# rock-slam/slam-pose_estimation

Hardware: NVIDIA B200
Metric: PoseUKF predict+update filter-steps/s (higher is better)
Workload: dtype f64

## Files before the change

slam_pose_estimation_b200/csrc/simt.cuh:

```cuda
#ifndef UKFB_SIMT_CUH
#define UKFB_SIMT_CUH

#ifndef UKFB_SIMT_EMU

#include <cuda_runtime.h>
#include <math.h>
#include <stdint.h>

#define UKFB_HD __host__ __device__ __forceinline__
#define UKFB_D __device__ __forceinline__
#define UKFB_DNI __device__ __noinline__
#define UKFB_GLOBAL __global__
#define UKFB_GRID_CONSTANT __grid_constant__
#define UKFB_CONSTANT __constant__
#define UKFB_LDCG(p) __ldcg(p)
#define UKFB_LAUNCH_BOUNDS(t, b) __launch_bounds__(t, b)
#define UKFB_SMEM_DECL extern __shared__ __align__(16) double ukfb_smem[];
#define UKFB_LDG(p) __ldg(p)
#define UKFB_UNROLL _Pragma("unroll")
#define UKFB_NOUNROLL _Pragma("unroll 1")

namespace ukfb {

UKFB_D void ukfb_sincos(double x, double* s, double* c) { sincos(x, s, c); }

UKFB_D void prefetch_l2(const void* p) { asm volatile("prefetch.global.L2 [%0];" ::"l"(p)); }

UKFB_D double warp_shfl(double v, int src) { return __shfl_sync(0xffffffffu, v, src); }

UKFB_D int hi_word(double x) { return __double2hiint(x); }

UKFB_D void pdl_launch_dependents() { asm volatile("griddepcontrol.launch_dependents;" ::: "memory"); }
UKFB_D void tile_done_add(unsigned long long* counter)
{
    asm volatile("red.release.gpu.global.add.u64 [%0], %1;" ::"l"(counter), "l"(1ull) : "memory");
}
UKFB_D void tile_done_wait(const unsigned long long* counter, unsigned long long need)
{
    unsigned long long v;
    for (unsigned spins = 0;; ++spins) {
        asm volatile("ld.acquire.gpu.global.u64 %0, [%1];" : "=l"(v) : "l"(counter) : "memory");
        if (v >= need) break;
        if (spins > 40000000u) __trap();
        __nanosleep(200);
    }
}

UKFB_D void warp_dmma(double& c0, double& c1, double a, double b)
{
    asm volatile("mma.sync.aligned.m8n8k4.row.col.f64.f64.f64.f64 {%0,%1}, {%2}, {%3}, {%0,%1};"
                 : "+d"(c0), "+d"(c1)
                 : "d"(a), "d"(b));
}

#ifndef UKFB_SEED_REFINEMENTS
#define UKFB_SEED_REFINEMENTS 2
#endif
UKFB_D double fast_rcp(double x)
{
    double y;
    asm("rcp.approx.ftz.f64 %0, %1;" : "=d"(y) : "d"(x));
    double e = fma(-x, y, 1.0);
    y = fma(y, e, y);
#if UKFB_SEED_REFINEMENTS >= 3
    e = fma(-x, y, 1.0);
    y = fma(y, e, y);
#endif
    e = fma(-x, y, 1.0);
    return fma(y, e, y);
}

UKFB_D void fast_sqrt_rsqrt(double x, double& s, double& r)
{
    double y;
    asm("rsqrt.approx.ftz.f64 %0, %1;" : "=d"(y) : "d"(x));
    double g = x * y, h = 0.5 * y;
    double e = fma(-g, h, 0.5);
    g = fma(g, e, g), h = fma(h, e, h);
#if UKFB_SEED_REFINEMENTS >= 3
    e = fma(-g, h, 0.5);
    g = fma(g, e, g), h = fma(h, e, h);
#endif
    e = fma(-g, h, 0.5);
    g = fma(g, e, g), h = fma(h, e, h);
    const double d = fma(-g, g, x);
    s = fma(d, h, g);
    r = h + h;
}

}

#else

#include <cmath>
#include <cstdint>

#include "simt_emu_rt.hpp"

#define UKFB_HD inline
#define UKFB_D inline
#define UKFB_DNI inline
#define UKFB_GLOBAL
#define UKFB_GRID_CONSTANT
#define UKFB_CONSTANT static const
#define UKFB_LDCG(p) (*(p))
#define UKFB_LAUNCH_BOUNDS(t, b)
#define UKFB_SMEM_DECL double* ukfb_smem = ::simt_emu::smem_base();
#define UKFB_LDG(p) (*(p))
#define UKFB_UNROLL
#define UKFB_NOUNROLL

namespace ukfb {
using std::atan;
using std::fabs;
using std::fma;
using std::sqrt;
inline void prefetch_l2(const void*) {}
inline int hi_word(double x)
{
    long long b;
    static_assert(sizeof(b) == sizeof(x), "");
    __builtin_memcpy(&b, &x, sizeof(b));
    return int(b >> 32);
}
inline void pdl_launch_dependents() {}
inline void tile_done_add(unsigned long long* counter) { __atomic_fetch_add(counter, 1ull, __ATOMIC_RELEASE); }
inline void tile_done_wait(const unsigned long long* counter, unsigned long long need)
{
    while (__atomic_load_n(counter, __ATOMIC_ACQUIRE) < need) {
    }
}
inline void ukfb_sincos(double x, double* s, double* c)
{
    *s = std::sin(x);
    *c = std::cos(x);
}
inline double warp_shfl(double v, int src)
{
    double* x = ::simt_emu::warp_xchg();
    const int lane = threadIdx.x & 31;
    x[lane] = v;
    __syncwarp();
    const double r = x[src & 31];
    __syncwarp();
    return r;
}
inline void warp_dmma(double& c0, double& c1, double a, double b)
{
    double* x = ::simt_emu::warp_xchg();
    const int lane = threadIdx.x & 31;
    x[lane] = a;
    x[32 + lane] = b;
    __syncwarp();
    const int row = lane >> 2, col = 2 * (lane & 3);
    for (int k = 0; k < 4; ++k) {
        c0 += x[row * 4 + k] * x[32 + col * 4 + k];
        c1 += x[row * 4 + k] * x[32 + (col + 1) * 4 + k];
    }
    __syncwarp();
}
inline double fast_rcp(double x) { return 1.0 / x; }
inline void fast_sqrt_rsqrt(double x, double& s, double& r)
{
    s = std::sqrt(x);
    r = 1.0 / s;
}
}

#endif

#endif
```

slam_pose_estimation_b200/csrc/ukf_batch.cu:

```cuda
#include <cuda_runtime.h>

#include <algorithm>
#include <cassert>
#include <cfloat>
#include <cmath>
#include <vector>
#include <cstdarg>
#include <cstdio>
#include <cstring>
#include <new>
#include <condition_variable>
#include <functional>
#include <mutex>
#include <string>
#include <thread>
#include <utility>

#include "ukf_device.cuh"
#include "ukf_thread.cuh"
#include "ukf_index.cuh"
#ifndef UKFB_DEFAULT_PREFETCH_BYTES
#define UKFB_DEFAULT_PREFETCH_BYTES 128
#endif
#ifndef UKFB_DEFAULT_WPB
// ... 332 lines not shown
        double v = 0.0;
        if (k < MU)
            v = mu[b * MU + k];
        else {
            const int e = k - MU;
            int r = 0;
            while ((r + 1) * (r + 2) / 2 <= e) ++r;
            const int c = e - r * (r + 1) / 2;
            v = sigma[(b * n + r) * n + c];
        }
        state[rec_index(tiled, b, k, REC)] = v;
    }
}

__global__ void unpack_mu_kernel(const double* __restrict__ state, double* __restrict__ mu, long long B, int MU, int REC, int tiled)
{
    const long long total = B * MU;
    for (long long i = blockIdx.x * (long long)blockDim.x + threadIdx.x; i < total; i += (long long)gridDim.x * blockDim.x) {
        const long long b = i / MU;
        const int k = int(i - b * MU);
        mu[i] = state[rec_index(tiled, b, k, REC)];
    }
}

__global__ void unpack_sigma_kernel(const double* __restrict__ state, double* __restrict__ sigma, long long B, int n, int MU, int REC, int tiled)
{
    const long long total = B * n * n;
    for (long long i = blockIdx.x * (long long)blockDim.x + threadIdx.x; i < total; i += (long long)gridDim.x * blockDim.x) {
        const long long b = i / (n * n);
        const int e = int(i - b * n * n);
        int r = e / n, c = e - (e / n) * n;
        if (c > r) {
            const int t = r;
            r = c;
            c = t;
        }
        sigma[i] = state[rec_index(tiled, b, MU + tri(r, c), REC)];
    }
}

__global__ void pack_rbs_kernel(double* __restrict__ state, const double* __restrict__ rbs, long long B, int tiled)
{
    const long long total = B * PoseF::REC;
    for (long long i = blockIdx.x * (long long)blockDim.x + threadIdx.x; i < total; i += (long long)gridDim.x * blockDim.x) {
        const long long b = i / PoseF::REC;
        const int k = int(i - b * PoseF::REC);
        const double* r = rbs + b * UKFB_RBS_DOUBLES;
        double v = 0.0;
        if (k < PoseF::MU)
            v = r[k];
        else {
            const int e = k - PoseF::MU;
            int row = 0;
            while ((row + 1) * (row + 2) / 2 <= e) ++row;
            const int col = e - row * (row + 1) / 2;
            if (row / 3 == col / 3) v = r[13 + (row / 3) * 9 + (row % 3) * 3 + (col % 3)];
        }
        state[rec_index(tiled, b, k, PoseF::REC)] = v;
    }
}

__global__ void unpack_rbs_kernel(const double* __restrict__ state, double* __restrict__ rbs, long long B, int tiled)
{
    const long long total = B * UKFB_RBS_DOUBLES;
    for (long long i = blockIdx.x * (long long)blockDim.x + threadIdx.x; i < total; i += (long long)gridDim.x * blockDim.x) {
        const long long b = i / UKFB_RBS_DOUBLES;
        const int k = int(i - b * UKFB_RBS_DOUBLES);
        double v;
        if (k >= 7 && k < 10) {
            double q[4], bv[3], nv[3];
            for (int j = 0; j < 4; ++j) q[j] = state[rec_index(tiled, b, 3 + j, PoseF::REC)];
            for (int j = 0; j < 3; ++j) bv[j] = state[rec_index(tiled, b, 7 + j, PoseF::REC)];
            quat_rotate(q, bv, nv);
            v = nv[k - 7];
        } else if (k < PoseF::MU)
            v = state[rec_index(tiled, b, k, PoseF::REC)];
        else {
            const int blk = (k - 13) / 9, e = (k - 13) % 9;
            int row = blk * 3 + e / 3, col = blk * 3 + e % 3;
            if (col > row) {
                const int t = row;
                row = col;
                col = t;
            }
            v = state[rec_index(tiled, b, PoseF::MU + tri(row, col), PoseF::REC)];
        }
        rbs[i] = v;
    }
}

__global__ void pack_q_kernel(double* __restrict__ Qp, const double* __restrict__ Q, long long count, int n, int LP)
{
    const long long total = count * LP;
    for (long long i = blockIdx.x * (long long)blockDim.x + threadIdx.x; i < total; i += (long long)gridDim.x * blockDim.x) {
        const long long b = i / LP;
        const int e = int(i - b * LP);
        int r = 0;
        while ((r + 1) * (r + 2) / 2 <= e) ++r;
        const int c = e - r * (r + 1) / 2;
        Qp[i] = Q[(b * n + r) * n + c];
    }
}

__global__ void unpack_q_kernel(const double* __restrict__ Qp, double* __restrict__ Q, long long count, int n, int LP, long long q_stride)
{
    const long long total = count * n * n;
    for (long long i = blockIdx.x * (long long)blockDim.x + threadIdx.x; i < total; i += (long long)gridDim.x * blockDim.x) {
        const long long b = i / (n * n);
        const int e = int(i - b * n * n);
        int r = e / n, c = e - (e / n) * n;
        if (c > r) {
            const int t = r;
            r = c;
            c = t;
        }
        Q[i] = Qp[b * q_stride + tri(r, c)];
    }
}

template <typename T>
__global__ void fill_kernel(T* __restrict__ dst, long long count, T v)
{
    for (long long i = blockIdx.x * (long long)blockDim.x + threadIdx.x; i < count; i += (long long)gridDim.x * blockDim.x) dst[i] = v;
}

__global__ void eye3_kernel(double* __restrict__ dst, long long count)
{
    for (long long i = blockIdx.x * (long long)blockDim.x + threadIdx.x; i < count; i += (long long)gridDim.x * blockDim.x)
        dst[i] = ((i % 9) % 4 == 0) ? 1.0 : 0.0;
}

__global__ void store_vec3_kernel(double* __restrict__ dst_mu, double* __restrict__ dst_cov, const double* __restrict__ mu,
                                  const double* __restrict__ cov, long long cov_stride, const uint8_t* __restrict__ mask,
                                  uint32_t* __restrict__ status, int check, long long B)
{
    for (long long b = blockIdx.x * (long long)blockDim.x + threadIdx.x; b < B; b += (long long)gridDim.x * blockDim.x) {
        if (mask && !mask[b]) continue;
        const double m0 = mu[b * 3], m1 = mu[b * 3 + 1], m2 = mu[b * 3 + 2];
        double c[9];
        for (int i = 0; i < 9; ++i) c[i] = cov ? cov[b * cov_stride + i] : ((i % 4 == 0) ? 1.0 : 0.0);
        if (check) {
            bool ok = isfinite(m0) && isfinite(m1) && isfinite(m2);
            for (int i = 0; i < 9; ++i) ok = ok && isfinite(c[i]);
            if (!ok) {
                status[b] |= UKFB_STATUS_NONFINITE_MEAS;
                continue;
            }
        }
        dst_mu[b * 3] = m0, dst_mu[b * 3 + 1] = m1, dst_mu[b * 3 + 2] = m2;
        if (dst_cov)
            for (int i = 0; i < 9; ++i) dst_cov[b * 9 + i] = c[i];
    }
}

__global__ void rotation_rate_kernel(const double* __restrict__ state, const double* __restrict__ gyro, double e0, double e1,
                                     double e2, const double* __restrict__ ori_params, double* __restrict__ out, long long B, int tiled)
{
    for (long long b = blockIdx.x * (long long)blockDim.x + threadIdx.x; b < B; b += (long long)gridDim.x * blockDim.x) {
        double q[4];
        for (int i = 0; i < 4; ++i) q[i] = state[rec_index(tiled, b, i, OriF::REC)];
        double e[3] = {e0, e1, e2};
        if (ori_params) e[0] = ori_params[b * 5 + 2], e[1] = ori_params[b * 5 + 3], e[2] = ori_params[b * 5 + 4];
        double r[3];
        quat_inv_rotate(q, e, r);
        for (int i = 0; i < 3; ++i) out[b * 3 + i] = gyro[b * 3 + i] - state[rec_index(tiled, b, 7 + i, OriF::REC)] - r[i];
    }
}

__global__ void ori_default_imu_kernel(const double* __restrict__ state, double* __restrict__ acc, double* __restrict__ gyro,
                                       long long B, int tiled)
{
    for (long long b = blockIdx.x * (long long)blockDim.x + threadIdx.x; b < B; b += (long long)gridDim.x * blockDim.x) {
        acc[b * 3] = 0.0, acc[b * 3 + 1] = 0.0, acc[b * 3 + 2] = state[rec_index(tiled, b, 13, OriF::REC)];
        gyro[b * 3] = gyro[b * 3 + 1] = gyro[b * 3 + 2] = 0.0;
    }
}

__global__ void status_summary_kernel(const uint32_t* __restrict__ status, long long B, long long* __restrict__ out)
{
    long long n = 0;
    unsigned bits = 0;
    for (long long b = blockIdx.x * (long long)blockDim.x + threadIdx.x; b < B; b += (long long)gridDim.x * blockDim.x) {
        const uint32_t s = status[b];
        n += s != 0;
        bits |= s;
    }
    for (int o = 16; o; o >>= 1) {
        n += __shfl_xor_sync(0xffffffffu, n, o);
        bits |= __shfl_xor_sync(0xffffffffu, bits, o);
    }
    if ((threadIdx.x & 31) == 0) {
        if (n) atomicAdd(reinterpret_cast<unsigned long long*>(out), (unsigned long long)n);
        if (bits) atomicOr(reinterpret_cast<unsigned long long*>(out + 1), (unsigned long long)bits);
    }
}

__global__ void __launch_bounds__(256) dfma_peak_kernel(double* out, int iters, double a, double b)
{
    double x0 = threadIdx.x, x1 = x0 + 1, x2 = x0 + 2, x3 = x0 + 3, x4 = x0 + 4, x5 = x0 + 5, x6 = x0 + 6, x7 = x0 + 7;
    for (int i = 0; i < iters; ++i) {
#pragma unroll
        for (int u = 0; u < 8; ++u) {
            x0 = fma(x0, a, b), x1 = fma(x1, a, b), x2 = fma(x2, a, b), x3 = fma(x3, a, b);
            x4 = fma(x4, a, b), x5 = fma(x5, a, b), x6 = fma(x6, a, b), x7 = fma(x7, a, b);
        }
    }
    const double s = ((x0 + x1) + (x2 + x3)) + ((x4 + x5) + (x6 + x7));
    if (s == 12345.678) out[0] = s;
}

static inline int grid_for(long long count, int block = 256)
{
    long long g = (count + block - 1) / block;
    if (g < 1) g = 1;
    if (g > 148 * 16) g = 148 * 16;
    return int(g);
}

struct EnvKnobs {
    int fast_wpb;
    long smem_pad_kb;
    int prefetch_bytes;
    long long prefetch_tiles;
    bool overlap;
    int overlap_max_waves;
    int overlap_min_waves_pct;
    EnvKnobs()
    {
        const char* e = getenv("UKFB_FAST_WPB");
        const int v = e ? atoi(e) : UKFB_DEFAULT_WPB;
        fast_wpb = (v == 1 || v == 2 || v == 4) ? v : UKFB_DEFAULT_WPB;
        e = getenv("UKFB_SMEM_PAD_KB");
        smem_pad_kb = e ? atol(e) : 0;
        e = getenv("UKFB_PREFETCH_BYTES");
        prefetch_bytes = e && atoi(e) >= 8 ? atoi(e) : UKFB_DEFAULT_PREFETCH_BYTES;
        e = getenv("UKFB_PREFETCH_TILES");
        prefetch_tiles = e ? atoll(e) : -1;
        e = getenv("UKFB_OVERLAP_LAUNCHES");
        overlap = e ? atoi(e) != 0 : true;
        e = getenv("UKFB_OVERLAP_MAX_WAVES");
        overlap_max_waves = e && atoi(e) > 0 ? atoi(e) : 12;
        e = getenv("UKFB_OVERLAP_MIN_WAVES_PCT");
        overlap_min_waves_pct = e ? atoi(e) : 100;
    }
};
static const EnvKnobs& knobs()
{
    static const EnvKnobs k;
    return k;
}

static std::mutex g_attr_mu;
template <class K>
static cudaError_t ensure_smem_attr(K kernel, int device, size_t smem)
{
    static std::vector<std::pair<const void*, int>> done;
    const std::pair<const void*, int> key(reinterpret_cast<const void*>(kernel), device);
    std::lock_guard<std::mutex> lock(g_attr_mu);
    for (const auto& d : done)
        if (d == key) return cudaSuccess;
    cudaError_t e = cudaFuncSetAttribute(kernel, cudaFuncAttributeMaxDynamicSharedMemorySize, int(smem));
    if (e == cudaSuccess) done.push_back(key);
    return e;
}

template <class F, int G, int WPB, int MINB>
static cudaError_t launch_step_t(const ukfb_handle* h, const StepParams& p)
{
    const size_t smem = sizeof(double) * WPB * Smem<F, G>::TOTAL;
    cudaError_t e = ensure_smem_attr(ukf_step_kernel<F, G, WPB, MINB>, h->device, smem);
    if (e != cudaSuccess) return e;
    const long long per_block = (long long)WPB * G;
    const long long grid = (p.B + per_block - 1) / per_block;
    ukf_step_kernel<F, G, WPB, MINB><<<unsigned(grid), WPB * 32, smem, h->stream>>>(p);
    return cudaGetLastError();
}

template <class F>
static cudaError_t launch_step_f(const ukfb_handle* h, const StepParams& p)
{
    switch (h->G * 100 + h->WPB * 10 + h->MINB) {
        case 443: return launch_step_t<F, 4, 4, 3>(h, p);
        case 444: return launch_step_t<F, 4, 4, 4>(h, p);
        case 1642: return launch_step_t<F, 16, 4, 2>(h, p);
        case 1652: return launch_step_t<F, 16, 5, 2>(h, p);
        case 842: return launch_step_t<F, 8, 4, 2>(h, p);
        case 844: return launch_step_t<F, 8, 4, 4>(h, p);
        default: return launch_step_t<F, 8, 4, 3>(h, p);
    }
}

template <class F>
static cudaError_t launch_thread_f(const ukfb_handle* h, const StepParams& p)
{
    const size_t smem = sizeof(double) * TSmem<F>::TOTAL;
    cudaError_t e = ensure_smem_attr(ukf_thread_kernel<F>, h->device, smem);
    if (e != cudaSuccess) return e;
    const long long grid = (p.B + TILE - 1) / TILE;
    ukf_thread_kernel<F><<<unsigned(grid), TILE, smem, h->stream>>>(p);
    return cudaGetLastError();
}

template <class K>
static cudaError_t launch_fast(K kernel, K kernel_overlap, int per_lane, ukfb_handle* h, const StepParams& p, ukfb_handle::FastCfg& cfg)
{
    const EnvKnobs& kn = knobs();
    const int wpb = kn.fast_wpb;
    const size_t smem = sizeof(double) * per_lane * TILE * wpb + size_t(kn.smem_pad_kb) * 1024;
    if (!cfg.attr_set) {
        cudaError_t e = ensure_smem_attr(kernel, h->device, smem);
        if (e == cudaSuccess) e = ensure_smem_attr(kernel_overlap, h->device, smem);
        if (e != cudaSuccess) return e;
        cfg.attr_set = true;
    }
    const long long tiles = (p.B + TILE - 1) / TILE;
    const long long grid = (tiles + wpb - 1) / wpb;
    StepParams q = p;
    if (cfg.prefetch_tiles < 0) {
        int per_sm = 0, sms = 0;
        if (cudaOccupancyMaxActiveBlocksPerMultiprocessor(&per_sm, kernel, TILE * wpb, smem) != cudaSuccess) per_sm = 0;
        if (cudaDeviceGetAttribute(&sms, cudaDevAttrMultiProcessorCount, h->device) != cudaSuccess) sms = 0;
        cfg.resident_warps = (long long)per_sm * wpb * sms;
        long long r = kn.prefetch_tiles;
        if (r < 0) {
            r = cfg.resident_warps / 4;
            if (r < 32 && per_sm > 0) r = 32;
        }
        cfg.prefetch_tiles = r > 0 ? r : 0;
    }
    q.prefetch_tiles = cfg.prefetch_tiles;
    q.prefetch_bytes = kn.prefetch_bytes;
    const bool overlap = kn.overlap && cfg.resident_warps > 0 && grid * wpb * 100 > kn.overlap_min_waves_pct * cfg.resident_warps &&
                         grid * wpb <= kn.overlap_max_waves * cfg.resident_warps;
    q.tile_done = overlap ? h->tile_done : nullptr;
    q.launch_seq = h->fast_launches + 1;
    cudaLaunchConfig_t lc;
    memset(&lc, 0, sizeof(lc));
    lc.gridDim = dim3(unsigned(grid));
    lc.blockDim = dim3(TILE * wpb);
    lc.dynamicSmemBytes = smem;
    lc.stream = h->stream;
    cudaLaunchAttribute at[1];
    at[0].id = cudaLaunchAttributeProgrammaticStreamSerialization;
    at[0].val.programmaticStreamSerializationAllowed = 1;
    lc.attrs = at;
    lc.numAttrs = overlap ? 1 : 0;
    const cudaError_t e = cudaLaunchKernelEx(&lc, overlap ? kernel_overlap : kernel, q);
    if (e != cudaSuccess) return e;
    if (overlap) h->fast_launches++;
    return cudaGetLastError();
}

static cudaError_t launch_pose_fast(ukfb_handle* h, const StepParams& p, bool may_have_orientation_meas)
{
    if (may_have_orientation_meas) return launch_fast(ukf_pose_fast_kernel<true, false>, ukf_pose_fast_kernel<true, true>, PF_PER_LANE, h, p, h->fast_cfg[1]);
    return launch_fast(ukf_pose_fast_kernel<false, false>, ukf_pose_fast_kernel<false, true>, PF_PER_LANE, h, p, h->fast_cfg[0]);
}

static cudaError_t launch_ori_fast(ukfb_handle* h, const StepParams& p)
{
    if (p.ori_params) return launch_fast(ukf_ori_fast_kernel<true, false>, ukf_ori_fast_kernel<true, true>, OF_PER_LANE, h, p, h->fast_cfg[1]);
    return launch_fast(ukf_ori_fast_kernel<false, false>, ukf_ori_fast_kernel<false, true>, OF_PER_LANE, h, p, h->fast_cfg[0]);
}

static int launch_step(ukfb_handle* h, const StepParams& p)
{
    cudaError_t e;
    if (h->tiled && h->fast && h->kind == UKFB_POSE) {
        bool ori_meas = p.do_update && (p.kind == UKFB_MEAS_POSE_ORIENTATION || p.kind == -2 || p.events);
        if (p.do_update && p.tick_kinds) ori_meas = h->tick_kinds_have_orientation;
        e = launch_pose_fast(h, p, ori_meas);
    }
    else if (h->tiled && h->fast)
        e = launch_ori_fast(h, p);
    else if (h->tiled)
        e = h->kind == UKFB_POSE ? launch_thread_f<PoseF>(h, p) : launch_thread_f<OriF>(h, p);
    else
        e = h->kind == UKFB_POSE ? launch_step_f<PoseF>(h, p) : launch_step_f<OriF>(h, p);
    if (e != cudaSuccess) return fail(UKFB_ERR_CUDA, "ukf_step_kernel launch: %s", cudaGetErrorString(e));
    h->launches++;
    return UKFB_OK;
}

static StepParams base_params(const ukfb_handle* h)
{
    StepParams p;
    memset(&p, 0, sizeof(p));
    p.state = h->state;
    p.Q = h->Q;
    p.q_stride = h->q_per_filter ? h->LP : 0;
    p.q_diagonal = h->q_per_filter ? 0 : h->q_diagonal;
    p.B = h->B;
    p.status = h->status;
    p.t_last = h->t_last;
    p.hist = h->hist;
    p.min_dt = h->min_dt;
    p.max_dt = h->max_dt;
    p.acc_mu = h->acc_mu;
    p.acc_cov = h->acc_cov;
    p.gyro_mu = h->gyro_mu;
    p.neg_inv_tau_g = -1.0 / h->tau_g;
    p.neg_inv_tau_a = -1.0 / h->tau_a;
    p.earth[0] = h->earth[0], p.earth[1] = h->earth[1], p.earth[2] = h->earth[2];
    p.kind = -1;
    p.K = 1;
    p.gate_d2 = h->gate_d2;
    p.ori_params = h->ori_params;
    return p;
}

static bool kind_ok(const ukfb_handle* h, int kind)
{
    if (h->kind == UKFB_POSE) return kind >= 0 && kind <= 8;
    return kind == UKFB_MEAS_ORI_VELOCITY;
}

#define NEED_INIT_AS(h, who) \
    if (!(h)->initialized) return fail(UKFB_ERR_NOT_INITIALIZED, "%s: filter not initialized", who)
#define NEED_INIT(h) NEED_INIT_AS(h, __func__)

extern "C" int ukfb_create(int filter_kind, int64_t batch, int device, ukfb_handle** out)
{
    if (!out) return fail(UKFB_ERR_INVALID, "ukfb_create: out is null");
    *out = nullptr;
    if (filter_kind != UKFB_POSE && filter_kind != UKFB_ORIENTATION) return fail(UKFB_ERR_INVALID, "ukfb_create: bad filter kind %d", filter_kind);
    if (batch < 1) return fail(UKFB_ERR_INVALID, "ukfb_create: batch must be >= 1");
    int ndev = 0;
    cudaError_t e = cudaGetDeviceCount(&ndev);
    if (e != cudaSuccess || ndev == 0)
        return fail(UKFB_ERR_CUDA, "ukfb_create: no CUDA device (%s); this engine has no CPU path", cudaGetErrorString(e));
    if (device < 0 || device >= ndev) return fail(UKFB_ERR_INVALID, "ukfb_create: device %d out of range (%d devices)", device, ndev);
    cudaDeviceProp prop;
    CU(cudaGetDeviceProperties(&prop, device));
    if (prop.major < 10) return fail(UKFB_ERR_CUDA, "ukfb_create: device %d is sm_%d%d; the kernels are built for sm_100a only", device, prop.major, prop.minor);

    ukfb_handle* h = new (std::nothrow) ukfb_handle;
    if (!h) return fail(UKFB_ERR_NOMEM, "ukfb_create: out of host memory");
    h->kind = filter_kind;
    h->device = device;
    h->B = batch;
    if (filter_kind == UKFB_POSE)
        h->n = PoseF::N, h->MU = PoseF::MU, h->LP = PoseF::LP, h->REC = PoseF::REC;
    else
        h->n = OriF::N, h->MU = OriF::MU, h->LP = OriF::LP, h->REC = OriF::REC;
    if (const char* g = getenv("UKFB_GROUP")) {
        const int G = atoi(g);
        if (G == 4 || G == 8 || G == 16) h->G = G;
    }
    if (const char* g = getenv("UKFB_KERNEL")) {
        h->tiled = strcmp(g, "warp") != 0;
        if (strcmp(g, "thread") == 0) h->fast = 0;
    }
    if (const char* g = getenv("UKFB_WARP_WPB")) h->WPB = atoi(g);
    if (const char* g = getenv("UKFB_MINB")) h->MINB = atoi(g);
    Bind bind_(h);
    if (!bind_.ok) {
        delete h;
        return fail(UKFB_ERR_CUDA, "ukfb_create: cudaSetDevice(%d) failed", device);
    }
#define CUH(call)                                                                     \
    do {                                                                              \
        cudaError_t e_ = (call);                                                      \
        if (e_ != cudaSuccess) {                                                      \
            fail(e_ == cudaErrorMemoryAllocation ? UKFB_ERR_NOMEM : UKFB_ERR_CUDA, "%s: %s", #call, cudaGetErrorString(e_)); \
            ukfb_destroy(h);                                                          \
            return e_ == cudaErrorMemoryAllocation ? UKFB_ERR_NOMEM : UKFB_ERR_CUDA; \
        }                                                                             \
    } while (0)
    const long long B = batch;
    CUH(cudaStreamCreateWithFlags(&h->stream, cudaStreamNonBlocking));
    const long long Bpad = (B + TILE - 1) / TILE * TILE;
    CUH(cudaMalloc(&h->state, sizeof(double) * Bpad * h->REC));
    CUH(cudaMalloc(&h->Q, sizeof(double) * h->LP));
    CUH(cudaMalloc(&h->status, sizeof(uint32_t) * B));
    CUH(cudaMalloc(&h->t_last, sizeof(long long) * B));
    CUH(cudaMalloc(&h->hist, sizeof(unsigned long long) * HIST_SLOTS * 8));
    CUH(cudaMalloc(&h->acc_mu, sizeof(double) * B * 3));
    CUH(cudaMalloc(&h->acc_cov, sizeof(double) * B * 9));
    CUH(cudaMalloc(&h->gyro_mu, sizeof(double) * B * 3));
    CUH(cudaMalloc(&h->summary, sizeof(long long) * 2));
    CUH(cudaMalloc(&h->tile_done, sizeof(unsigned long long) * (Bpad / TILE)));
    CUH(cudaMemsetAsync(h->tile_done, 0, sizeof(unsigned long long) * (Bpad / TILE), h->stream));
    CUH(cudaMemsetAsync(h->state, 0, sizeof(double) * Bpad * h->REC, h->stream));
    CUH(cudaMemsetAsync(h->status, 0, sizeof(uint32_t) * B, h->stream));
    CUH(cudaMemsetAsync(h->t_last, 0, sizeof(long long) * B, h->stream));
    CUH(cudaMemsetAsync(h->hist, 0, sizeof(unsigned long long) * HIST_SLOTS * 8, h->stream));
    CUH(cudaMemsetAsync(h->gyro_mu, 0, sizeof(double) * B * 3, h->stream));
    {
        double q[OriF::LP];
        for (int i = 0; i < OriF::LP; ++i) q[i] = 0.0;
        if (filter_kind == UKFB_POSE) {
            const double d[4] = {UKFB_POSE_Q_POSITION, UKFB_POSE_Q_ORIENTATION, UKFB_POSE_Q_VELOCITY, UKFB_POSE_Q_ANGULAR_VELOCITY};
            for (int i = 0; i < 12; ++i) q[tri(i, i)] = d[i / 3];
        }
        CUH(cudaMemcpyAsync(h->Q, q, sizeof(double) * h->LP, cudaMemcpyHostToDevice, h->stream));
        CUH(cudaStreamSynchronize(h->stream));
        h->q_diagonal = 2;
    }
    fill_kernel<double><<<grid_for(B * 3), 256, 0, h->stream>>>(h->acc_mu, B * 3, filter_kind == UKFB_POSE ? double(NAN) : 0.0);
    eye3_kernel<<<grid_for(B * 9), 256, 0, h->stream>>>(h->acc_cov, B * 9);
    for (int i = 0; i < 16; ++i) CUH(cudaEventCreate(&h->ev[i]));
    CUH(cudaGetLastError());
    CUH(cudaStreamSynchronize(h->stream));
#undef CUH
    *out = h;
    return UKFB_OK;
}

extern "C" int ukfb_create_sharded(int filter_kind, int64_t batch, const int* devices, int n_devices, ukfb_handle** out)
{
    if (!out) return fail(UKFB_ERR_INVALID, "ukfb_create_sharded: out is null");
    *out = nullptr;
    if (filter_kind != UKFB_POSE && filter_kind != UKFB_ORIENTATION) return fail(UKFB_ERR_INVALID, "ukfb_create_sharded: bad filter kind %d", filter_kind);
    if (n_devices < 1 || n_devices > 64) return fail(UKFB_ERR_INVALID, "ukfb_create_sharded: n_devices must be 1..64");
    if (batch < n_devices) return fail(UKFB_ERR_INVALID, "ukfb_create_sharded: batch must be >= n_devices (every shard holds at least one filter)");
    ukfb_handle* h = new (std::nothrow) ukfb_handle;
    if (!h) return fail(UKFB_ERR_NOMEM, "ukfb_create_sharded: out of host memory");
    h->kind = filter_kind;
    h->B = batch;
    if (filter_kind == UKFB_POSE)
        h->n = PoseF::N, h->MU = PoseF::MU, h->LP = PoseF::LP, h->REC = PoseF::REC;
    else
        h->n = OriF::N, h->MU = OriF::MU, h->LP = OriF::LP, h->REC = OriF::REC;
    const long long base = batch / n_devices, extra = batch % n_devices;
    h->first.assign(size_t(n_devices) + 1, 0);
    for (int i = 0; i < n_devices; ++i) h->first[size_t(i) + 1] = h->first[size_t(i)] + base + (i < extra ? 1 : 0);
    for (int i = 0; i < n_devices; ++i) {
        ukfb_handle* sh = nullptr;
        const int rc = ukfb_create(filter_kind, h->first[size_t(i) + 1] - h->first[size_t(i)], devices ? devices[i] : i, &sh);
        if (rc) {
            for (ukfb_handle* made : h->shards) ukfb_destroy(made);
            delete h;
            return rc;
        }
        h->shards.push_back(sh);
    }
    h->device = h->shards[0]->device;
    h->tiled = h->shards[0]->tiled, h->fast = h->shards[0]->fast;
    h->pool = new (std::nothrow) ShardPool(n_devices);
    if (!h->pool) {
        for (ukfb_handle* made : h->shards) ukfb_destroy(made);
        delete h;
        return fail(UKFB_ERR_NOMEM, "ukfb_create_sharded: out of host memory");
    }
    *out = h;
    return UKFB_OK;
}

extern "C" int ukfb_shard_count(const ukfb_handle* h) { return !h ? 0 : (is_sharded(h) ? int(h->shards.size()) : 1); }

extern "C" int ukfb_shard(ukfb_handle* h, int i, ukfb_handle** shard, int64_t* first, int64_t* count)
{
    if (!h) return fail(UKFB_ERR_INVALID, "ukfb_shard: null handle");
    const int n = ukfb_shard_count(h);
    if (i < 0 || i >= n) return fail(UKFB_ERR_INVALID, "ukfb_shard: shard %d out of range (%d shards)", i, n);
    if (shard) *shard = is_sharded(h) ? h->shards[size_t(i)] : h;
    if (first) *first = is_sharded(h) ? h->first[size_t(i)] : 0;
    if (count) *count = is_sharded(h) ? h->first[size_t(i) + 1] - h->first[size_t(i)] : h->B;
    return UKFB_OK;
}

extern "C" int ukfb_host_alloc(void** ptr, uint64_t bytes)
{
    if (!ptr || !bytes) return fail(UKFB_ERR_INVALID, "ukfb_host_alloc: bad argument");
    *ptr = nullptr;
    cudaError_t e = cudaHostAlloc(ptr, size_t(bytes), cudaHostAllocPortable);
    if (e != cudaSuccess) return fail(e == cudaErrorMemoryAllocation ? UKFB_ERR_NOMEM : UKFB_ERR_CUDA, "ukfb_host_alloc(%llu bytes): %s", (unsigned long long)bytes, cudaGetErrorString(e));
    return UKFB_OK;
}

extern "C" int ukfb_host_free(void* ptr)
{
    if (!ptr) return UKFB_OK;
    CU(cudaFreeHost(ptr));
    return UKFB_OK;
}

extern "C" int ukfb_destroy(ukfb_handle* h)
{
    if (!h) return UKFB_OK;
    if (is_sharded(h)) {
        delete h->pool;
        for (ukfb_handle* s : h->shards) ukfb_destroy(s);
        delete h;
        return UKFB_OK;
    }
    Bind bind_(h);
    if (h->stream) cudaStreamSynchronize(h->stream);
    cudaFree(h->state), cudaFree(h->Q), cudaFree(h->status), cudaFree(h->t_last), cudaFree(h->hist), cudaFree(h->tile_done), cudaFree(h->tick_kinds_dev);
    cudaFree(h->acc_mu), cudaFree(h->acc_cov), cudaFree(h->gyro_mu), cudaFree(h->stage), cudaFree(h->summary), cudaFree(h->ori_params);
    for (int k = 0; k < UKFB_MEAS_KIND_COUNT; ++k) cudaFree(h->meas_cov[k]);
    for (int i = 0; i < 16; ++i)
        if (h->ev[i]) cudaEventDestroy(h->ev[i]);
    if (h->pipe.made) {
        cudaStreamSynchronize(h->pipe.s_in), cudaStreamSynchronize(h->pipe.s_out);
        for (int i = 0; i < 2; ++i) {
            cudaFree(h->pipe.in[i]), cudaFree(h->pipe.out[i]);
            cudaEventDestroy(h->pipe.in_ready[i]), cudaEventDestroy(h->pipe.in_consumed[i]);
            cudaEventDestroy(h->pipe.out_ready[i]), cudaEventDestroy(h->pipe.out_drained[i]);
        }
        cudaStreamDestroy(h->pipe.s_in), cudaStreamDestroy(h->pipe.s_out);
    }
    if (h->stream) cudaStreamDestroy(h->stream);
    delete h;
    return UKFB_OK;
}

extern "C" int64_t ukfb_batch(const ukfb_handle* h) { return h ? h->B : 0; }
extern "C" int ukfb_dof(const ukfb_handle* h) { return h ? h->n : 0; }
extern "C" int ukfb_mu_size(const ukfb_handle* h) { return h ? h->MU : 0; }
extern "C" int ukfb_device(const ukfb_handle* h) { return h ? h->device : -1; }
extern "C" int ukfb_is_initialized(const ukfb_handle* h) { return h && h->initialized ? 1 : 0; }

static int initialize_dev(ukfb_handle* h, const double* d_mu, const double* d_sigma)
{
    pack_kernel<<<grid_for(h->B * h->REC), 256, 0, h->stream>>>(h->state, d_mu, d_sigma, h->B, h->n, h->MU, h->LP, h->REC, h->tiled);
    CU(cudaGetLastError());
    CU(cudaMemsetAsync(h->t_last, 0, sizeof(long long) * h->B, h->stream));
    if (h->kind == UKFB_ORIENTATION && h->first_init) {
        ori_default_imu_kernel<<<grid_for(h->B), 256, 0, h->stream>>>(h->state, h->acc_mu, h->gyro_mu, h->B, h->tiled);
        CU(cudaGetLastError());
    }
    h->first_init = false;
    h->initialized = true;
    return UKFB_OK;
}

extern "C" int ukfb_initialize(ukfb_handle* h, const double* mu, const double* sigma)
{
    CHECK_H(h);
    if (!mu || !sigma) return fail(UKFB_ERR_INVALID, "ukfb_initialize: null argument");
    if (is_sharded(h)) {
        const int rc = fan_out(h, [&](ukfb_handle* s_, long long f_, long long) { return ukfb_initialize(s_, mu + f_ * s_->MU, sigma + f_ * s_->n * s_->n); });
        if (rc == UKFB_OK) h->initialized = true;
        return rc;
    }
    const double *d_mu, *d_sigma;
    Staging st(h, false);
    st.in(&d_mu, mu, sizeof(double) * h->B * h->MU);
    st.in(&d_sigma, sigma, sizeof(double) * h->B * h->n * h->n);
    int rc = st.commit();
    if (!rc) rc = initialize_dev(h, d_mu, d_sigma);
    return rc ? rc : st.finish();
}

extern "C" int ukfb_initialize_from_body_states_dev(ukfb_handle* h, const double* d_rbs)
{
    CHECK_H(h);
    UKFB_NOT_SHARDED(h);
    if (h->kind != UKFB_POSE) return fail(UKFB_ERR_INVALID, "ukfb_initialize_from_body_states: BodyStateMeasurement belongs to PoseUKF");
    if (!d_rbs) return fail(UKFB_ERR_INVALID, "ukfb_initialize_from_body_states: null argument");
    pack_rbs_kernel<<<grid_for(h->B * h->REC), 256, 0, h->stream>>>(h->state, d_rbs, h->B, h->tiled);
    CU(cudaGetLastError());
    CU(cudaMemsetAsync(h->t_last, 0, sizeof(long long) * h->B, h->stream));
    h->first_init = false;
    h->initialized = true;
    return UKFB_OK;
}

extern "C" int ukfb_initialize_from_body_states(ukfb_handle* h, const double* rbs)
{
    CHECK_H(h);
    if (!rbs) return fail(UKFB_ERR_INVALID, "ukfb_initialize_from_body_states: null argument");
    if (is_sharded(h)) {
        if (h->kind != UKFB_POSE) return fail(UKFB_ERR_INVALID, "ukfb_initialize_from_body_states: BodyStateMeasurement belongs to PoseUKF");
// ... 1239 lines not shown
```

slam_pose_estimation_b200/csrc/ukf_pose_fast.cuh:

```cuda
#ifndef UKFB_POSE_FAST_CUH
#define UKFB_POSE_FAST_CUH

#include "ukf_thread.cuh"

namespace ukfb {

#define UKFB_PS(e) sm[(e) * TILE + lane]

#ifndef UKFB_PF_MEAN_UNROLL
#define UKFB_PF_MEAN_UNROLL 1
#endif
#ifndef UKFB_PF_COV_UNROLL
#define UKFB_PF_COV_UNROLL 1
#endif
#ifndef UKFB_PF_MIN_BLOCKS
#define UKFB_PF_MIN_BLOCKS 2
#endif
#ifndef UKFB_PF_MAX_THREADS
#define UKFB_PF_MAX_THREADS (4 * TILE)
#endif
#define UKFB_PRAGMA_(x) _Pragma(#x)
#ifdef UKFB_SIMT_EMU
#define UKFB_LOOP_UNROLL(n)
#else
// ... 50 lines not shown
    const double n2 = q[0] * q[0] + q[1] * q[1] + q[2] * q[2] + q[3] * q[3];
    return fabs(n2 - 1.0) <= PF_QNORM_TOL;
}

UKFB_D void pf_rotate(const double* q, const double* v, double* out)
{
    const double ux = fma(q[1], v[2], -(q[2] * v[1]));
    const double uy = fma(q[2], v[0], -(q[0] * v[2]));
    const double uz = fma(q[0], v[1], -(q[1] * v[0]));
    out[0] = fma(2.0, fma(q[3], ux, fma(q[1], uz, -(q[2] * uy))), v[0]);
    out[1] = fma(2.0, fma(q[3], uy, fma(q[2], ux, -(q[0] * uz))), v[1]);
    out[2] = fma(2.0, fma(q[3], uz, fma(q[0], uy, -(q[1] * ux))), v[2]);
}

UKFB_D void pf_matvec(const double* Rm, const double* v, double* out)
{
    out[0] = Rm[0] * v[0] + Rm[1] * v[1] + Rm[2] * v[2];
    out[1] = Rm[3] * v[0] + Rm[4] * v[1] + Rm[5] * v[2];
    out[2] = Rm[6] * v[0] + Rm[7] * v[1] + Rm[8] * v[2];
}

struct D2 {
    double a, b;
    UKFB_D D2() {}
    UKFB_D explicit D2(double x) : a(x), b(x) {}
    UKFB_D D2(double x, double y) : a(x), b(y) {}
};
UKFB_D D2 operator+(D2 x, D2 y) { return D2(x.a + y.a, x.b + y.b); }
UKFB_D D2 operator-(D2 x, D2 y) { return D2(x.a - y.a, x.b - y.b); }
UKFB_D D2 operator*(D2 x, D2 y) { return D2(x.a * y.a, x.b * y.b); }
UKFB_D D2 operator-(D2 x) { return D2(-x.a, -x.b); }
UKFB_D D2 operator+(D2 x, double y) { return D2(x.a + y, x.b + y); }
UKFB_D D2 operator-(D2 x, double y) { return D2(x.a - y, x.b - y); }
UKFB_D D2 operator*(D2 x, double y) { return D2(x.a * y, x.b * y); }
UKFB_D D2 operator*(double x, D2 y) { return D2(x * y.a, x * y.b); }
UKFB_D D2 operator+(double x, D2 y) { return D2(x + y.a, x + y.b); }
UKFB_D double tfma(double x, double y, double z) { return fma(x, y, z); }
UKFB_D D2 tfma(D2 x, D2 y, D2 z) { return D2(fma(x.a, y.a, z.a), fma(x.b, y.b, z.b)); }
UKFB_D D2 tfma(double x, D2 y, D2 z) { return D2(fma(x, y.a, z.a), fma(x, y.b, z.b)); }
UKFB_D D2 tfma(D2 x, double y, D2 z) { return D2(fma(x.a, y, z.a), fma(x.b, y, z.b)); }
UKFB_D D2 tfma(D2 x, D2 y, double z) { return D2(fma(x.a, y.a, z), fma(x.b, y.b, z)); }
UKFB_D D2 tfma(double x, D2 y, double z) { return D2(fma(x, y.a, z), fma(x, y.b, z)); }
UKFB_D D2 tfma(D2 x, double y, double z) { return D2(fma(x.a, y, z), fma(x.b, y, z)); }
UKFB_D D2 tfma(double x, double y, D2 z) { return D2(fma(x, y, z.a), fma(x, y, z.b)); }
UKFB_D bool all_le(D2 x, double lim) { return (x.a <= lim) && (x.b <= lim); }
#define UKFB_TPOLY5(C, v, v2) tfma(tfma(C[5], v, C[4]), (v2) * (v2), tfma(tfma(C[3], v, C[2]), v2, tfma(C[1], v, C[0])))

UKFB_D void pf_exp(const D2* v, double scale, D2* q, bool& slow)
{
    const double half = scale * 0.5;
    const D2 norm2 = v[0] * v[0] + v[1] * v[1] + v[2] * v[2];
    const D2 x2 = (half * half) * norm2;
    slow = slow || !(pf_exp_in_range(x2.a) && pf_exp_in_range(x2.b));
    const D2 x4 = x2 * x2;
    const D2 c = UKFB_TPOLY5(SO3_COS5_C, x2, x4);
    const D2 mult = UKFB_TPOLY5(SO3_SINC5_C, x2, x4) * half;
    q[0] = mult * v[0];
    q[1] = mult * v[1];
    q[2] = mult * v[2];
    q[3] = c;
}

UKFB_D D2 two_asin_over_s_poly(D2 y)
{
    const D2 y2 = y * y, y4 = y2 * y2;
    const D2 p01 = tfma(SO3_ASIN_C[1], y, SO3_ASIN_C[0]), p23 = tfma(SO3_ASIN_C[3], y, SO3_ASIN_C[2]);
    const D2 p45 = tfma(SO3_ASIN_C[5], y, SO3_ASIN_C[4]), p67 = tfma(SO3_ASIN_C[7], y, SO3_ASIN_C[6]);
    const D2 q0 = tfma(p23, y2, p01), q1 = tfma(p67, y2, p45);
    return tfma(tfma(SO3_ASIN_C[8], y4, q1), y4, q0);
}

UKFB_D void pf_log(const D2* q, D2* out, bool& slow)
{
    const D2 nv2 = q[0] * q[0] + q[1] * q[1] + q[2] * q[2];
    const D2 w = q[3];
    const D2 d = tfma(w, w, nv2) - 1.0;
    slow = slow || !(pf_log_in_range(w.a) && pf_log_in_range(w.b));
    const D2 s0 = two_asin_over_s_poly(tfma(-nv2, d, nv2));
    const D2 s = tfma(s0, -0.5 * d, s0);
    out[0] = s * q[0];
    out[1] = s * q[1];
    out[2] = s * q[2];
}

UKFB_D void pf_rotate(const D2* q, const D2* v, D2* out)
{
    const D2 ux = tfma(q[1], v[2], -(q[2] * v[1]));
    const D2 uy = tfma(q[2], v[0], -(q[0] * v[2]));
    const D2 uz = tfma(q[0], v[1], -(q[1] * v[0]));
    out[0] = tfma(2.0, tfma(q[3], ux, tfma(q[1], uz, -(q[2] * uy))), v[0]);
    out[1] = tfma(2.0, tfma(q[3], uy, tfma(q[2], ux, -(q[0] * uz))), v[1]);
    out[2] = tfma(2.0, tfma(q[3], uz, tfma(q[0], uy, -(q[1] * ux))), v[2]);
}

template <class B>
UKFB_D void quat_mul(const D2* a, const B* b, D2* r)
{
    r[3] = a[3] * b[3] - a[0] * b[0] - a[1] * b[1] - a[2] * b[2];
    r[0] = a[3] * b[0] + a[0] * b[3] + a[1] * b[2] - a[2] * b[1];
    r[1] = a[3] * b[1] + a[1] * b[3] + a[2] * b[0] - a[0] * b[2];
    r[2] = a[3] * b[2] + a[2] * b[3] + a[0] * b[1] - a[1] * b[0];
}
template <class B>
UKFB_D void quat_mul_conj(const D2* a, const B* b, D2* r)
{
    r[3] = a[3] * b[3] + a[0] * b[0] + a[1] * b[1] + a[2] * b[2];
    r[0] = -a[3] * b[0] + a[0] * b[3] - a[1] * b[2] + a[2] * b[1];
    r[1] = -a[3] * b[1] + a[1] * b[3] - a[2] * b[0] + a[0] * b[2];
    r[2] = -a[3] * b[2] + a[2] * b[3] - a[0] * b[1] + a[1] * b[0];
}

#ifndef UKFB_PF_WIDE_CALLS
#define UKFB_PF_WIDE_CALLS 1
#endif
constexpr double PF_EXP_WIDE_X2 = 10.24;
#ifndef UKFB_PF_WIDE_TRACE
#define UKFB_PF_WIDE_TRACE 1.0
#endif
constexpr double PF_WIDE_TRACE = UKFB_PF_WIDE_TRACE;
#define UKFB_TPOLY6(C, v, v2) \
    tfma(tfma(C[6], v2, tfma(C[5], v, C[4])), (v2) * (v2), tfma(tfma(C[3], v, C[2]), v2, tfma(C[1], v, C[0])))
UKFB_D bool all_le(double x, double lim) { return x <= lim; }
UKFB_D double v_sign(double w) { return w < 0.0 ? -1.0 : 1.0; }
UKFB_D D2 v_sign(D2 w) { return D2(v_sign(w.a), v_sign(w.b)); }
UKFB_D void v_sqrt_rsqrt(double x, double& sq, double& rs) { fast_sqrt_rsqrt(x, sq, rs); }
UKFB_D void v_sqrt_rsqrt(D2 x, D2& sq, D2& rs)
{
    fast_sqrt_rsqrt(x.a, sq.a, rs.a);
    fast_sqrt_rsqrt(x.b, sq.b, rs.b);
}

template <class V>
UKFB_D void pf_exp_wide(const V* v, double scale, V* q, bool& hard)
{
    const double half = scale * 0.5;
    const V norm2 = v[0] * v[0] + v[1] * v[1] + v[2] * v[2];
    const V x2 = (half * half) * norm2;
    hard = hard || !all_le(x2, PF_EXP_WIDE_X2);
    const V y2 = x2 * (1.0 / 64.0), y4 = y2 * y2;
    V w = UKFB_TPOLY6(SO3_COS_C, y2, y4);
    const V mult = UKFB_TPOLY6(SO3_SINC_C, y2, y4) * (half * 0.125);
    V a = mult * v[0], b = mult * v[1], c = mult * v[2];
    UKFB_UNROLL
    for (int k = 0; k < 3; ++k) {
        const V t = w + w, n = a * a + b * b + c * c;
        w = tfma(w, w, -n);
        a = t * a, b = t * b, c = t * c;
    }
    q[0] = a, q[1] = b, q[2] = c, q[3] = w;
}

template <class V>
UKFB_D void pf_log_wide(const V* q, V* out)
{
    V x = q[0], y = q[1], z = q[2], w = q[3];
    const V n2 = tfma(w, w, x * x + y * y + z * z);
    const V k = v_sign(w) * tfma(n2 - 1.0, -0.5, 1.0);
    x = x * k, y = y * k, z = z * k, w = w * k;
    UKFB_UNROLL
    for (int i = 0; i < 3; ++i) {
        V c, rc;
        v_sqrt_rsqrt((w + 1.0) * 0.5, c, rc);
        const V h = rc * 0.5;
        x = x * h, y = y * h, z = z * h, w = c;
    }
    const V nv2 = x * x + y * y + z * z;
    const V d = tfma(w, w, nv2) - 1.0;
    const V s0 = two_asin_over_s_poly(tfma(-nv2, d, nv2));
    const V sc = tfma(s0, -0.5 * d, s0) * 8.0;
    out[0] = sc * x, out[1] = sc * y, out[2] = sc * z;
}

template <class V> struct PfV3 { V v[3]; };
template <class V> struct PfQ4 { V q[4]; bool hard; };
#if UKFB_PF_WIDE_CALLS
template <class V>
UKFB_DNI PfQ4<V> pf_exp_wide_call(PfV3<V> v, double scale)
{
    PfQ4<V> r;
    r.hard = false;
    pf_exp_wide<V>(v.v, scale, r.q, r.hard);
    return r;
}
template <class V>
UKFB_DNI PfV3<V> pf_log_wide_call(PfQ4<V> q)
{
    PfV3<V> r;
    pf_log_wide<V>(q.q, r.v);
    return r;
}
template <class V>
UKFB_D void pf_exp_wide_shared(const V* v, double scale, V* q, bool& hard)
{
    PfV3<V> a;
    a.v[0] = v[0], a.v[1] = v[1], a.v[2] = v[2];
    const PfQ4<V> r = pf_exp_wide_call<V>(a, scale);
    q[0] = r.q[0], q[1] = r.q[1], q[2] = r.q[2], q[3] = r.q[3];
    hard = hard || r.hard;
}
template <class V>
UKFB_D void pf_log_wide_shared(const V* q, V* out)
{
    PfQ4<V> a;
    a.q[0] = q[0], a.q[1] = q[1], a.q[2] = q[2], a.q[3] = q[3], a.hard = false;
    const PfV3<V> r = pf_log_wide_call<V>(a);
    out[0] = r.v[0], out[1] = r.v[1], out[2] = r.v[2];
}
#else
template <class V>
UKFB_D void pf_exp_wide_shared(const V* v, double scale, V* q, bool& hard) { pf_exp_wide<V>(v, scale, q, hard); }
template <class V>
UKFB_D void pf_log_wide_shared(const V* q, V* out) { pf_log_wide<V>(q, out); }
#endif

template <bool WIDE>
UKFB_D void pf_exp1(const double* v, double scale, double* q, bool& slow)
{
    if (WIDE)
        pf_exp_wide_shared<double>(v, scale, q, slow);
    else
        pf_exp(v, scale, q, slow);
}
template <bool WIDE>
UKFB_D void pf_log1(const double* q, double* out, bool& slow)
{
    if (WIDE)
        pf_log_wide_shared<double>(q, out);
    else
        pf_log(q, out, slow);
}

template <int NCOL>
UKFB_D bool pf_cholesky(double* a)
{
    bool ok = true;
    UKFB_UNROLL
    for (int j = 0; j < NCOL; ++j) {
        double ajj = a[tri(j, j)];
        UKFB_UNROLL
        for (int k = 0; k < j; ++k) ajj -= a[tri(j, k)] * a[tri(j, k)];
        if (!pivot_ok(ajj)) {
            ok = false;
            ajj = 1.0;
        }
        double d, rinv;
        fast_sqrt_rsqrt(ajj, d, rinv);
        a[tri(j, j)] = d;
        UKFB_UNROLL
        for (int i = j + 1; i < 12; ++i) {
            double s = a[tri(i, j)];
            UKFB_UNROLL
            for (int k = 0; k < j; ++k) s -= a[tri(i, k)] * a[tri(j, k)];
            a[tri(i, j)] = s * rinv;
        }
    }
    return ok;
}

struct TrueT { static constexpr bool value = true; };
struct FalseT { static constexpr bool value = false; };

struct PoseMu {
    double p[3], q[4], v[3], w[3];
};

template <class F>
UKFB_D void prefetch_next_wave(const StepParams& p, long long tile, int lane)
{
    if (p.prefetch_tiles <= 0) return;
    const long long nt = tile + p.prefetch_tiles;
    if ((nt + 1) * TILE > p.B) return;
    const char* rec = reinterpret_cast<const char*>(p.state + nt * (TILE * F::REC));
    const int bytes = TILE * F::REC * int(sizeof(double));
    UKFB_NOUNROLL
    for (int o = lane * p.prefetch_bytes; o < bytes; o += TILE * p.prefetch_bytes) prefetch_l2(rec + o);
    const long long nb = nt * TILE;
    const int o = lane * p.prefetch_bytes;
    if (p.acc_mu && o < TILE * 24) prefetch_l2(reinterpret_cast<const char*>(p.acc_mu + nb * 3) + o);
    if (F::KIND == 1 && p.gyro_mu && o < TILE * 24) prefetch_l2(reinterpret_cast<const char*>(p.gyro_mu + nb * 3) + o);
    if (p.do_update && p.z && o < TILE * 8 * p.z_stride) prefetch_l2(reinterpret_cast<const char*>(p.z + nb * p.z_stride) + o);
    if (p.do_update && p.R && p.r_stride > 0 && o < TILE * 8 * p.r_stride)
        prefetch_l2(reinterpret_cast<const char*>(p.R + nb * p.r_stride) + o);
    if (p.do_predict && !p.time_mode && p.dt && o < TILE * 8 * p.dt_stride) prefetch_l2(reinterpret_cast<const char*>(p.dt + nb * p.dt_stride) + o);
}

template <bool WIDE, class V>
UKFB_D void pf_exp_t(const V* v, double scale, V* q, bool& flag)
{
    if (WIDE)
        pf_exp_wide_shared<V>(v, scale, q, flag);
    else
        pf_exp(v, scale, q, flag);
}
template <bool WIDE, class V>
UKFB_D void pf_log_t(const V* q, V* out, bool& flag)
{
    if (WIDE)
        pf_log_wide_shared<V>(q, out);
    else
        pf_log(q, out, flag);
}


template <bool WIDE>
UKFB_D void pf_point2(const D2* qs, const D2* ps, const D2* vs, const D2* ws, double dt, const double* ref_p, const double* ref_q,
                      D2* d, bool& slow)
{
    D2 rv[3], e[4], qn[4], r[4];
    pf_rotate(qs, vs, rv);
    pf_exp_t<WIDE>(ws, dt, e, slow);
    quat_mul(qs, e, qn);
    d[0] = tfma(dt, rv[0], ps[0]) - ref_p[0];
    d[1] = tfma(dt, rv[1], ps[1]) - ref_p[1];
    d[2] = tfma(dt, rv[2], ps[2]) - ref_p[2];
    quat_mul_conj(qn, ref_q, r);
    pf_log_t<WIDE>(r, d + 3, slow);
}

template <bool WIDE>
UKFB_D void pf_pair_a(const double* sm, int lane, int j, const PoseMu& m, const double* vm, double dt, const double* ref_p,
                      const double* ref_q, double* L, double* dpl, double* dmi, bool& slow)
{
    UKFB_UNROLL
    for (int i = 0; i < 12; ++i) L[i] = UKFB_PS(PF_LA + j * 12 + i);
    double e[4];
    pf_exp_t<WIDE>(L + 3, 1.0, e, slow);
    const double* q = m.q;
    const double t0 = e[0] * q[3] + e[1] * q[2] - e[2] * q[1];
    const double t1 = e[1] * q[3] + e[2] * q[0] - e[0] * q[2];
    const double t2 = e[2] * q[3] + e[0] * q[1] - e[1] * q[0];
    const double t3 = -(e[0] * q[0] + e[1] * q[1] + e[2] * q[2]);
    const D2 qs[4] = {D2(fma(e[3], q[0], t0), fma(e[3], q[0], -t0)), D2(fma(e[3], q[1], t1), fma(e[3], q[1], -t1)),
                      D2(fma(e[3], q[2], t2), fma(e[3], q[2], -t2)), D2(fma(e[3], q[3], t3), fma(e[3], q[3], -t3))};
    const D2 ps[3] = {D2(m.p[0] + L[0], m.p[0] - L[0]), D2(m.p[1] + L[1], m.p[1] - L[1]), D2(m.p[2] + L[2], m.p[2] - L[2])};
    const D2 vs[3] = {D2(vm[0] + L[6], vm[0] - L[6]), D2(vm[1] + L[7], vm[1] - L[7]), D2(vm[2] + L[8], vm[2] - L[8])};
    const D2 ws[3] = {D2(m.w[0] + L[9], m.w[0] - L[9]), D2(m.w[1] + L[10], m.w[1] - L[10]), D2(m.w[2] + L[11], m.w[2] - L[11])};
    D2 d[6];
    pf_point2<WIDE>(qs, ps, vs, ws, dt, ref_p, ref_q, d, slow);
    UKFB_UNROLL
    for (int i = 0; i < 6; ++i) dpl[i] = d[i].a, dmi[i] = d[i].b;
}

template <bool WIDE>
UKFB_D void pf_pair_b(const double* sm, int lane, int j, const double* Rm, const double* rw0, const double* c, double dt,
                      double* L, double* dopl, double* domi, double* wv, bool& slow)
{
    UKFB_UNROLL
    for (int i = 0; i < 6; ++i) L[i] = UKFB_PS(PF_LB + (j - 6) * 6 + i);
    double u[3], rv[3];
    pf_matvec(Rm, L + 3, u);
    pf_matvec(Rm, L, rv);
    wv[0] = dt * rv[0], wv[1] = dt * rv[1], wv[2] = dt * rv[2];
    const D2 rw[3] = {D2(rw0[0] + u[0], rw0[0] - u[0]), D2(rw0[1] + u[1], rw0[1] - u[1]), D2(rw0[2] + u[2], rw0[2] - u[2])};
    D2 e[4], r[4], d[3];
    pf_exp_t<WIDE>(rw, dt, e, slow);
    quat_mul(e, c, r);
    pf_log_t<WIDE>(r, d, slow);
    UKFB_UNROLL
    for (int i = 0; i < 3; ++i) dopl[i] = d[i].a, domi[i] = d[i].b;
}

template <bool WIDE>
UKFB_D void pf_pair_d(const double* sm, int lane, int j, const double* delta, const double* c, double* dp, double* dn, bool& slow)
{
    D2 v[3], e[4], r2[4], d[3];
    UKFB_UNROLL
    for (int i = 0; i < 3; ++i) {
        const double l = UKFB_PS(PF_LA + j * 12 + 3 + i);
        v[i] = D2(delta[3 + i] + l, delta[3 + i] - l);
    }
    pf_exp_t<WIDE>(v, 1.0, e, slow);
    quat_mul(e, c, r2);
    pf_log_t<WIDE>(r2, d, slow);
    UKFB_UNROLL
    for (int i = 0; i < 3; ++i) dp[i] = d[i].a, dn[i] = d[i].b;
}

#ifndef UKFB_PF_WIDE_COLUMN_N2
#define UKFB_PF_WIDE_COLUMN_N2 0.2
#endif
constexpr double PF_WIDE_COLUMN_N2 = UKFB_PF_WIDE_COLUMN_N2;
template <bool WIDE>
UKFB_D void pf_pair_a_sel(const double* sm, int lane, int j, const PoseMu& m, const double* vm, double dt, const double* ref_p,
                          const double* ref_q, double* L, double* dpl, double* dmi, bool& slow)
{
    if (!WIDE) {
        pf_pair_a<false>(sm, lane, j, m, vm, dt, ref_p, ref_q, L, dpl, dmi, slow);
        return;
    }
    const double l3 = UKFB_PS(PF_LA + j * 12 + 3), l4 = UKFB_PS(PF_LA + j * 12 + 4), l5 = UKFB_PS(PF_LA + j * 12 + 5);
    bool redo = l3 * l3 + l4 * l4 + l5 * l5 > PF_WIDE_COLUMN_N2;
    if (!redo) pf_pair_a<false>(sm, lane, j, m, vm, dt, ref_p, ref_q, L, dpl, dmi, redo);
    if (redo) pf_pair_a<true>(sm, lane, j, m, vm, dt, ref_p, ref_q, L, dpl, dmi, slow);
}
template <bool WIDE>
UKFB_D void pf_pair_b_sel(const double* sm, int lane, int j, const double* Rm, const double* rw0, const double* c, double dt,
                          double* L, double* dopl, double* domi, double* wv, bool& slow)
{
    if (!WIDE) {
        pf_pair_b<false>(sm, lane, j, Rm, rw0, c, dt, L, dopl, domi, wv, slow);
        return;
    }
    bool redo = false;
    pf_pair_b<false>(sm, lane, j, Rm, rw0, c, dt, L, dopl, domi, wv, redo);
    if (redo) pf_pair_b<true>(sm, lane, j, Rm, rw0, c, dt, L, dopl, domi, wv, slow);
}
template <bool WIDE>
UKFB_D void pf_pair_d_sel(const double* sm, int lane, int j, const double* delta, const double* c, double* dp, double* dn, bool& slow)
{
    if (!WIDE) {
        pf_pair_d<false>(sm, lane, j, delta, c, dp, dn, slow);
        return;
    }
    const double l3 = UKFB_PS(PF_LA + j * 12 + 3), l4 = UKFB_PS(PF_LA + j * 12 + 4), l5 = UKFB_PS(PF_LA + j * 12 + 5);
    bool redo = l3 * l3 + l4 * l4 + l5 * l5 > PF_WIDE_COLUMN_N2;
    if (!redo) pf_pair_d<false>(sm, lane, j, delta, c, dp, dn, redo);
    if (redo) pf_pair_d<true>(sm, lane, j, delta, c, dp, dn, slow);
}

#ifdef UKFB_SIMT_EMU
inline unsigned long long pf_fallbacks[5] = {0, 0, 0, 0, 0};
#define UKFB_PF_COUNT(i) __atomic_fetch_add(&pf_fallbacks[i], 1ull, __ATOMIC_RELAXED)
#else
#define UKFB_PF_COUNT(i)
#endif
struct PfLit {
    PoseMu m;
    uint32_t status;
    int passes;
};

UKFB_D void pf_mu_to_slots(double* loc, const PoseMu& m)
{
    typedef TSmem<PoseF> TS;
    UKFB_UNROLL
    for (int i = 0; i < 3; ++i) {
        loc[TS::OFF_MU + i] = m.p[i];
        loc[TS::OFF_MU + 7 + i] = m.v[i];
        loc[TS::OFF_MU + 10 + i] = m.w[i];
    }
    UKFB_UNROLL
    for (int i = 0; i < 4; ++i) loc[TS::OFF_MU + 3 + i] = m.q[i];
}

UKFB_D void pf_mu_from_slots(const double* loc, PoseMu& m)
{
    typedef TSmem<PoseF> TS;
    UKFB_UNROLL
    for (int i = 0; i < 3; ++i) {
        m.p[i] = loc[TS::OFF_MU + i];
        m.v[i] = loc[TS::OFF_MU + 7 + i];
        m.w[i] = loc[TS::OFF_MU + 10 + i];
    }
    UKFB_UNROLL
    for (int i = 0; i < 4; ++i) m.q[i] = loc[TS::OFF_MU + 3 + i];
}

UKFB_DNI PfLit pf_literal_predict(double* sig, const double* Qp, const double* acov, ModelArgs ma, PoseMu m)
{
    typedef TSmem<PoseF> TS;
    UKFB_PF_COUNT(0);
    double loc[TS::PER_LANE];
    PfLit r;
    r.m = m, r.passes = 0;
    pf_mu_to_slots(loc, m);
    if (!cholesky_thread<PoseF, 1>(sig, loc, 0)) {
        r.status = UKFB_STATUS_NOT_SPD;
        return r;
    }
    store_noise<PoseF, 1>(loc, 0, sig, Qp, acov, ma);
    r.status = mean_and_cov<PoseF, true, 1>(loc, 0, sig, ma, &r.passes);
    UKFB_UNROLL
    for (int i = 0; i < PoseF::MU; ++i) loc[TS::OFF_MU + i] = loc[TS::OFF_REF + i];
    pf_mu_from_slots(loc, r.m);
    return r;
}

struct PfDelta {
    double d[12];
};

UKFB_DNI PfLit pf_literal_update(double* sig, int kind, const double* zm, const double* Rm, int r_ld, ModelArgs ma, PoseMu m,
                                 PfDelta delta, bool first, double gate_d2)
{
    typedef TSmem<PoseF> TS;
    UKFB_PF_COUNT(first ? 1 : 2);
    double loc[TS::PER_LANE];
    PfLit r;
    r.m = m, r.passes = 0, r.status = 0;
    pf_mu_to_slots(loc, m);
    if (first) {
        if (!cholesky_thread<PoseF, 1>(sig, loc, 0)) {
            r.status = UKFB_STATUS_NOT_SPD;
            return r;
        }
        r.status = update_first_half<PoseF, 1>(loc, 0, sig, kind, zm, Rm, r_ld, gate_d2);
        if (r.status & UKFB_STATUS_MEAS_REJECTED) return r;
    } else {
        UKFB_UNROLL
        for (int i = 0; i < 12; ++i) loc[TS::OFF_DELTA + i] = delta.d[i];
    }
    if (!cholesky_thread<PoseF, 1>(sig, loc, 0)) {
        r.status |= UKFB_STATUS_NOT_SPD;
        return r;
    }
    r.status |= mean_and_cov<PoseF, false, 1>(loc, 0, sig, ma, &r.passes);
    UKFB_UNROLL
    for (int i = 0; i < PoseF::MU; ++i) loc[TS::OFF_MU + i] = loc[TS::OFF_REF + i];
    pf_mu_from_slots(loc, r.m);
    return r;
}

template <bool WIDE>
UKFB_D bool pf_predict(int q_diagonal, double* sm, int lane, double* sig, double* a, const double* Qp, const double* acov,
                       const ModelArgs& ma, PoseMu& m, bool to_smem, uint32_t& status, int& passes_out, bool& spd)
{
    const double dt = ma.dt;
    if (!WIDE && a[tri(3, 3)] + a[tri(4, 4)] + a[tri(5, 5)] > PF_WIDE_TRACE) return false;
    {
        spd = pf_cholesky<12>(a);
        if (!spd) return true;
        UKFB_UNROLL
        for (int j = 0; j < 6; ++j) {
            UKFB_UNROLL
            for (int i = 0; i < 12; ++i) UKFB_PS(PF_LA + j * 12 + i) = i >= j ? a[tri(i, j)] : 0.0;
        }
        UKFB_UNROLL
        for (int j = 6; j < 12; ++j) {
            UKFB_UNROLL
            for (int i = 6; i < 12; ++i) UKFB_PS(PF_LB + (j - 6) * 6 + (i - 6)) = i >= j ? a[tri(i, j)] : 0.0;
        }
    }
    bool slow = !pf_unit(m.q);
    double Rm[9];
    quat_matrix(m.q, Rm);
    double vm[3] = {m.v[0], m.v[1], m.v[2]};
    if (ma.has_acc) {
        vm[0] = fma(dt, ma.acc[0], vm[0]);
        vm[1] = fma(dt, ma.acc[1], vm[1]);
        vm[2] = fma(dt, ma.acc[2], vm[2]);
    }
    double rw0[3], p0n[3], q0n[4];
    {
        double rv0[3], e0[4];
        pf_matvec(Rm, vm, rv0);
        pf_matvec(Rm, m.w, rw0);
        p0n[0] = fma(dt, rv0[0], m.p[0]);
        p0n[1] = fma(dt, rv0[1], m.p[1]);
        p0n[2] = fma(dt, rv0[2], m.p[2]);
        pf_exp1<WIDE>(rw0, dt, e0, slow);
        quat_mul(e0, m.q, q0n);
    }
    double ref_p[3] = {p0n[0], p0n[1], p0n[2]};
    double ref_q[4] = {q0n[0], q0n[1], q0n[2], q0n[3]};

    int it = 0, passes = 0;
    while (true) {
        double md[6];
        double d0[6];
        {
            double r[4];
            d0[0] = p0n[0] - ref_p[0], d0[1] = p0n[1] - ref_p[1], d0[2] = p0n[2] - ref_p[2];
            quat_mul_conj(q0n, ref_q, r);
            pf_log1<WIDE>(r, d0 + 3, slow);
        }
        md[0] = 13.0 * d0[0], md[1] = 13.0 * d0[1], md[2] = 13.0 * d0[2];
        md[3] = d0[3], md[4] = d0[4], md[5] = d0[5];
        UKFB_LOOP_UNROLL(UKFB_PF_MEAN_UNROLL)
        for (int j = 0; j < 6; ++j) {
            double L[12], dpl[6], dmi[6];
            pf_pair_a_sel<WIDE>(sm, lane, j, m, vm, dt, ref_p, ref_q, L, dpl, dmi, slow);
            UKFB_UNROLL
            for (int i = 0; i < 6; ++i) md[i] += dpl[i] + dmi[i];
        }
        double c[4];
        quat_mul_conj(m.q, ref_q, c);
        UKFB_LOOP_UNROLL(UKFB_PF_MEAN_UNROLL)
        for (int j = 6; j < 12; ++j) {
            double L[6], dopl[3], domi[3], wv[3];
            pf_pair_b_sel<WIDE>(sm, lane, j, Rm, rw0, c, dt, L, dopl, domi, wv, slow);
            UKFB_UNROLL
            for (int i = 0; i < 3; ++i) md[3 + i] += dopl[i] + domi[i];
        }
        double n2 = 0.0;
        UKFB_UNROLL
        for (int i = 0; i < 6; ++i) {
            md[i] = div_ns<PoseF::NS>(md[i]);
            n2 += md[i] * md[i];
        }
        ref_p[0] += md[0], ref_p[1] += md[1], ref_p[2] += md[2];
        {
            double e[4], r[4];
            pf_exp1<WIDE>(md + 3, 1.0, e, slow);
            quat_mul(e, ref_q, r);
            ref_q[0] = r[0], ref_q[1] = r[1], ref_q[2] = r[2], ref_q[3] = r[3];
        }
        ++passes;
        if (slow || !(n2 > UKFB_MEAN_TOL * UKFB_MEAN_TOL)) break;
        if (++it >= UKFB_MEAN_MAX_IT) {
            status |= UKFB_STATUS_MEAN_NO_CONVERGE;
            break;
        }
    }
    if (slow) return false;

    double C[21], X[36];
    {
        double d0[6], r[4];
        d0[0] = p0n[0] - ref_p[0], d0[1] = p0n[1] - ref_p[1], d0[2] = p0n[2] - ref_p[2];
        quat_mul_conj(q0n, ref_q, r);
        pf_log1<WIDE>(r, d0 + 3, slow);
        UKFB_UNROLL
        for (int i = 0; i < 6; ++i) {
            UKFB_UNROLL
            for (int k = 0; k <= i; ++k) C[tri(i, k)] = d0[i] * d0[k];
        }
        UKFB_LOOP_UNROLL(UKFB_PF_COV_UNROLL)
        for (int j = 0; j < 6; ++j) {
            double L[12], dpl[6], dmi[6];
            pf_pair_a_sel<WIDE>(sm, lane, j, m, vm, dt, ref_p, ref_q, L, dpl, dmi, slow);
            UKFB_UNROLL
            for (int i = 0; i < 6; ++i) {
                UKFB_UNROLL
                for (int k = 0; k <= i; ++k) C[tri(i, k)] = fma(dpl[i], dpl[k], fma(dmi[i], dmi[k], C[tri(i, k)]));
            }
            UKFB_UNROLL
            for (int k = 0; k < 6; ++k) UKFB_PS(PF_LA + j * 12 + k) = dpl[k] - dmi[k];
        }
        double Xb[18];
        UKFB_UNROLL
        for (int i = 0; i < 18; ++i) Xb[i] = 0.0;
        double c[4];
        quat_mul_conj(m.q, ref_q, c);
        UKFB_LOOP_UNROLL(UKFB_PF_COV_UNROLL)
        for (int j = 6; j < 12; ++j) {
            double L[6], dpl[6], dmi[6], wv[3];
            pf_pair_b_sel<WIDE>(sm, lane, j, Rm, rw0, c, dt, L, dpl + 3, dmi + 3, wv, slow);
            UKFB_UNROLL
            for (int i = 0; i < 3; ++i) dpl[i] = d0[i] + wv[i], dmi[i] = d0[i] - wv[i];
            UKFB_UNROLL
            for (int i = 0; i < 6; ++i) {
                UKFB_UNROLL
                for (int k = 0; k <= i; ++k) C[tri(i, k)] = fma(dpl[i], dpl[k], fma(dmi[i], dmi[k], C[tri(i, k)]));
            }
            UKFB_UNROLL
            for (int k = 0; k < 3; ++k) {
                const double dd = dpl[3 + k] - dmi[3 + k];
                UKFB_UNROLL
                for (int i = 0; i < 6; ++i) Xb[i * 3 + k] = fma(L[i], dd, Xb[i * 3 + k]);
            }
        }
        if (slow) return false;
        UKFB_UNROLL
        for (int i = 0; i < 6; ++i) {
            UKFB_UNROLL
            for (int k = 0; k < 3; ++k) X[i * 6 + k] = 0.0, X[i * 6 + 3 + k] = Xb[i * 3 + k];
        }
        UKFB_UNROLL
        for (int j = 0; j < 6; ++j) {
            double dd[6];
            UKFB_UNROLL
            for (int k = 0; k < 6; ++k) dd[k] = UKFB_PS(PF_LA + j * 12 + k);
            UKFB_UNROLL
            for (int i = 0; i < 6; ++i) {
                const double l = UKFB_PS(PF_LA + j * 12 + 6 + i);
                UKFB_UNROLL
                for (int k = 0; k < 6; ++k) X[i * 6 + k] = fma(l, dd[k], X[i * 6 + k]);
            }
        }
        UKFB_UNROLL
        for (int j = 6; j < 9; ++j) {
            double Lc[6], rv[3];
            UKFB_UNROLL
            for (int i = 0; i < 6; ++i) Lc[i] = i >= j - 6 ? UKFB_PS(PF_LB + (j - 6) * 6 + i) : 0.0;
            pf_matvec(Rm, Lc, rv);
            UKFB_UNROLL
            for (int k = 0; k < 3; ++k) {
                const double dd = 2.0 * (dt * rv[k]);
                UKFB_UNROLL
                for (int i = j - 6; i < 6; ++i) X[i * 6 + k] = fma(Lc[i], dd, X[i * 6 + k]);
            }
        }
    }

    auto commit = [&](auto qv, auto iso) {
        const double scale = ma.has_acc ? 1.0 : dt;
        double nb[12], na[6];
        UKFB_UNROLL
        for (int i = 0; i < 12; ++i) nb[i] = 0.0;
        UKFB_UNROLL
        for (int i = 0; i < 6; ++i) na[i] = 0.0;
        if (!ma.has_acc && decltype(iso)::value) {
            nb[tri(0, 0)] = nb[tri(1, 1)] = nb[tri(2, 2)] = scale * qv(0, 0);
            nb[6 + tri(0, 0)] = nb[6 + tri(1, 1)] = nb[6 + tri(2, 2)] = scale * qv(3, 3);
        } else if (!ma.has_acc) {
            UKFB_UNROLL
            for (int blk = 0; blk < 2; ++blk) {
                const int off = blk * 3;
                double t[9];
                UKFB_UNROLL
                for (int r = 0; r < 3; ++r) {
                    UKFB_UNROLL
                    for (int k = 0; k < 3; ++k) {
                        double s = 0.0;
                        UKFB_UNROLL
                        for (int l = 0; l < 3; ++l) s += Rm[r * 3 + l] * (l >= k ? qv(off + l, off + k) : qv(off + k, off + l));
                        t[r * 3 + k] = s;
                    }
                }
                UKFB_UNROLL
                for (int r = 0; r < 3; ++r) {
                    UKFB_UNROLL
                    for (int cc = 0; cc <= r; ++cc) {
                        double s = 0.0;
                        UKFB_UNROLL
                        for (int k = 0; k < 3; ++k) s += t[r * 3 + k] * Rm[cc * 3 + k];
                        nb[blk * 6 + tri(r, cc)] = scale * s;
                    }
                }
            }
        } else {
            UKFB_UNROLL
            for (int r = 0; r < 3; ++r) {
                UKFB_UNROLL
                for (int cc = 0; cc <= r; ++cc) na[tri(r, cc)] = 2.0 * acov[r * 3 + cc];
            }
        }
        UKFB_UNROLL
        for (int i = 0; i < 12; ++i) {
            UKFB_UNROLL
            for (int k = 0; k <= i; ++k) {
                const int e = tri(i, k);
                double nz = scale * qv(i, k);
                if (i < 6 && i / 3 == k / 3) nz = ma.has_acc ? nz : nb[(i / 3) * 6 + tri(i % 3, k % 3)];
                if (i >= 6 && i < 9 && k >= 6) nz = ma.has_acc ? na[tri(i - 6, k - 6)] : nz;
                double s;
                if (i < 6)
                    s = fma(0.5, C[e], nz);
                else if (k < 6)
                    s = fma(0.5, X[(i - 6) * 6 + k], nz);
                else
                    s = sig[e * TILE] + nz;
                sig[e * TILE] = s;
                if (to_smem) UKFB_PS(e) = s;
            }
        }
    };
    if (q_diagonal == 2)
        commit([&](int i, int k) { return i == k ? UKFB_LDG(Qp + tri(i, i)) : 0.0; }, TrueT());
    else if (q_diagonal)
        commit([&](int i, int k) { return i == k ? UKFB_LDG(Qp + tri(i, i)) : 0.0; }, FalseT());
    else
        commit([&](int i, int k) { return UKFB_LDG(Qp + tri(i, k)); }, FalseT());
    m.p[0] = ref_p[0], m.p[1] = ref_p[1], m.p[2] = ref_p[2];
    m.q[0] = ref_q[0], m.q[1] = ref_q[1], m.q[2] = ref_q[2], m.q[3] = ref_q[3];
    m.v[0] = vm[0], m.v[1] = vm[1], m.v[2] = vm[2];
    passes_out = passes;
    return true;
}

UKFB_DNI PfLit pf_predict_slow(double* sm, int lane, double* sig, const double* Qp, const double* acov, ModelArgs ma, PoseMu m,
                               int to_smem, int q_diagonal, int* in_smem)
{
    {
        double a[PoseF::LP];
        UKFB_UNROLL
        for (int e = 0; e < PoseF::LP; ++e) a[e] = sig[e * TILE];
        PfLit r;
        r.m = m, r.status = 0, r.passes = 0;
        bool spd = true;
        if (pf_predict<true>(q_diagonal, sm, lane, sig, a, Qp, acov, ma, r.m, to_smem != 0, r.status, r.passes, spd)) {
            UKFB_PF_COUNT(3);
            if (!spd) r.status |= UKFB_STATUS_NOT_SPD;
            *in_smem = spd ? to_smem : 0;
            return r;
        }
    }
    *in_smem = 0;
    return pf_literal_predict(sig, Qp, acov, ma, m);
}

UKFB_D int pf_sel(int kind, int c)
{
    switch (kind) {
        case 0: return c;
        case 1: return c < 2 ? c : -1;
        case 2: return c == 0 ? 2 : -1;
        case 4: return 6 + c;
        case 5: return c < 2 ? 6 + c : -1;
        case 6: return c == 0 ? 8 : -1;
        case 7: return c == 0 ? 6 : (c == 1 ? 11 : -1);
        default: return 9 + c;
    }
}

UKFB_D double pf_mu_tangent(const PoseMu& m, int t)
{
    double r = m.p[0];
    r = t == 1 ? m.p[1] : r;
    r = t == 2 ? m.p[2] : r;
    r = t == 6 ? m.v[0] : r;
    r = t == 7 ? m.v[1] : r;
    r = t == 8 ? m.v[2] : r;
    r = t == 9 ? m.w[0] : r;
    r = t == 10 ? m.w[1] : r;
    r = t == 11 ? m.w[2] : r;
    return r;
}

template <bool WIDE>
UKFB_D bool pf_apply_delta(double* sm, int lane, double* sig, PoseMu& m, const double* delta, uint32_t& status, int& passes_out, int& stage)
{
    bool slow = !pf_unit(m.q);
    const bool off_sphere = slow;
    bool lost_factor = false;
    double e0[4], q0n[4];
    pf_exp1<WIDE>(delta + 3, 1.0, e0, slow);
    quat_mul(e0, m.q, q0n);
    double ref_q[4] = {q0n[0], q0n[1], q0n[2], q0n[3]};
    int it = 0, passes = 0;
    while (true) {
        double c[4], r[4], d0[3], md[3];
        quat_mul_conj(m.q, ref_q, c);
        quat_mul(e0, c, r);
        pf_log1<WIDE>(r, d0, slow);
        md[0] = 13.0 * d0[0], md[1] = 13.0 * d0[1], md[2] = 13.0 * d0[2];
        UKFB_NOUNROLL
        for (int j = 0; j < 6; ++j) {
            double dp[3], dn[3];
            pf_pair_d_sel<WIDE>(sm, lane, j, delta, c, dp, dn, slow);
            md[0] += dp[0] + dn[0], md[1] += dp[1] + dn[1], md[2] += dp[2] + dn[2];
        }
        double n2 = 0.0;
        UKFB_UNROLL
        for (int i = 0; i < 3; ++i) {
            md[i] = div_ns<PoseF::NS>(md[i]);
            n2 += md[i] * md[i];
        }
        {
            double e[4], rr[4];
            pf_exp1<WIDE>(md, 1.0, e, slow);
            quat_mul(e, ref_q, rr);
            ref_q[0] = rr[0], ref_q[1] = rr[1], ref_q[2] = rr[2], ref_q[3] = rr[3];
        }
        ++passes;
        if (slow || !(n2 > UKFB_MEAN_TOL * UKFB_MEAN_TOL)) break;
        if (++it >= UKFB_MEAN_MAX_IT) {
            status |= UKFB_STATUS_MEAN_NO_CONVERGE;
            break;
        }
    }
    double Coo[6], Xc[27];
    if (!slow) {
        double c[4], r[4], d0[3];
        quat_mul_conj(m.q, ref_q, c);
        quat_mul(e0, c, r);
        pf_log1<WIDE>(r, d0, slow);
        UKFB_UNROLL
        for (int i = 0; i < 3; ++i) {
            UKFB_UNROLL
            for (int k = 0; k <= i; ++k) Coo[tri(i, k)] = 13.0 * d0[i] * d0[k];
        }
        bool late = false;
        UKFB_NOUNROLL
        for (int j = 0; j < 6; ++j) {
            double dp[3], dn[3];
            pf_pair_d_sel<WIDE>(sm, lane, j, delta, c, dp, dn, late);
            UKFB_UNROLL
            for (int i = 0; i < 3; ++i) {
                UKFB_UNROLL
                for (int k = 0; k <= i; ++k) Coo[tri(i, k)] = fma(dp[i], dp[k], fma(dn[i], dn[k], Coo[tri(i, k)]));
            }
            UKFB_UNROLL
            for (int k = 0; k < 3; ++k) UKFB_PS(PF_LA + j * 12 + 3 + k) = dp[k] - dn[k];
        }
        slow = slow || late;
        lost_factor = late;
        UKFB_UNROLL
        for (int i = 0; i < 27; ++i) Xc[i] = 0.0;
        UKFB_UNROLL
        for (int j = 0; j < 6; ++j) {
            double dd[3];
            UKFB_UNROLL
            for (int k = 0; k < 3; ++k) dd[k] = UKFB_PS(PF_LA + j * 12 + 3 + k);
            UKFB_UNROLL
            for (int t = 0; t < 9; ++t) {
                const int row = t < 3 ? t : t + 3;
                if (row < j) continue;
                const double l = UKFB_PS(PF_LA + j * 12 + row);
                UKFB_UNROLL
                for (int k = 0; k < 3; ++k) Xc[t * 3 + k] = fma(l, dd[k], Xc[t * 3 + k]);
            }
        }
    }
    if (slow) {
        stage = (WIDE || lost_factor || off_sphere) ? 1 : 2;
        return false;
    }
    UKFB_UNROLL
    for (int i = 0; i < 3; ++i) {
        UKFB_UNROLL
        for (int k = 0; k <= i; ++k) sig[tri(3 + i, 3 + k) * TILE] = 0.5 * Coo[tri(i, k)];
        UKFB_UNROLL
        for (int t = 0; t < 3; ++t) sig[tri(3 + i, t) * TILE] = 0.5 * Xc[t * 3 + i];
        UKFB_UNROLL
        for (int t = 3; t < 9; ++t) sig[tri(t + 3, 3 + i) * TILE] = 0.5 * Xc[t * 3 + i];
    }
    UKFB_UNROLL
    for (int i = 0; i < 3; ++i) {
        m.p[i] += delta[i];
        m.v[i] += delta[6 + i];
        m.w[i] += delta[9 + i];
    }
    m.q[0] = ref_q[0], m.q[1] = ref_q[1], m.q[2] = ref_q[2], m.q[3] = ref_q[3];
    passes_out = passes;
    return true;
}

template <bool ORI_MEAS>
UKFB_D bool pf_update(double* sm, int lane, double* sig, int kind, const double* zm, const double* Rmeas, int r_ld, PoseMu& m,
                      double* delta, uint32_t& status, int& passes_out, bool& spd, double gate_d2, int& stage)
{
    stage = 0;
    const int m_dim = meas_dim(kind);
    int sel[3];
    UKFB_UNROLL
    for (int c = 0; c < 3; ++c) sel[c] = pf_sel(kind, c);

    double Sxz[36], S[9], innov[3];
    if (ORI_MEAS) {
        bool slow = !pf_unit(m.q);
        double a[PoseF::LP];
        UKFB_UNROLL
        for (int e = 0; e < PoseF::LP; ++e) a[e] = UKFB_PS(e);
        spd = pf_cholesky<12>(a);
        if (!spd) return true;
        constexpr int PF_E = 78;
        UKFB_UNROLL
        for (int j = 0; j < 6; ++j) {
            double e[4];
            const double Lo[3] = {j <= 3 ? a[tri(3, j <= 3 ? j : 3)] : 0.0, j <= 4 ? a[tri(4, j <= 4 ? j : 4)] : 0.0, a[tri(5, j)]};
            pf_exp(Lo, 1.0, e, slow);
            UKFB_UNROLL
            for (int i = 0; i < 4; ++i) UKFB_PS(PF_E + 4 * j + i) = e[i];
        }
        double zin[4];
        {
            const double v[3] = {zm[0], zm[1], zm[2]};
            so3_exp(v, 1.0, zin);
        }
        double zref[4] = {m.q[0], m.q[1], m.q[2], m.q[3]};
        int it = 0;
        while (!slow) {
            double c[4], d0[3], md[3];
            quat_mul_conj(m.q, zref, c);
            pf_log(c, d0, slow);
            md[0] = 13.0 * d0[0], md[1] = 13.0 * d0[1], md[2] = 13.0 * d0[2];
            UKFB_NOUNROLL
            for (int j = 0; j < 6; ++j) {
                D2 e[4], r2[4], d[3];
                UKFB_UNROLL
                for (int i = 0; i < 4; ++i) {
                    const double x = UKFB_PS(PF_E + 4 * j + i);
                    e[i] = D2(x, i < 3 ? -x : x);
                }
                quat_mul(e, c, r2);
                pf_log(r2, d, slow);
                md[0] += d[0].a + d[0].b, md[1] += d[1].a + d[1].b, md[2] += d[2].a + d[2].b;
            }
            UKFB_UNROLL
            for (int i = 0; i < 3; ++i) md[i] = div_ns<PoseF::NS>(md[i]);
            const double n2 = md[0] * md[0] + md[1] * md[1] + md[2] * md[2];
            {
                double e[4], rr[4];
                pf_exp(md, 1.0, e, slow);
                quat_mul(e, zref, rr);
                zref[0] = rr[0], zref[1] = rr[1], zref[2] = rr[2], zref[3] = rr[3];
            }
            if (!(n2 > UKFB_MEAN_TOL * UKFB_MEAN_TOL)) break;
            if (++it >= UKFB_MEAN_MAX_IT) {
                status |= UKFB_STATUS_MEAN_NO_CONVERGE;
                break;
            }
        }
        {
            double c[4], d0[3];
            quat_mul_conj(m.q, zref, c);
            pf_log(c, d0, slow);
            UKFB_UNROLL
            for (int r = 0; r < 3; ++r) {
                UKFB_UNROLL
                for (int cc = 0; cc < 3; ++cc) S[r * 3 + cc] = 13.0 * d0[r] * d0[cc];
            }
            UKFB_NOUNROLL
            for (int j = 0; j < 6; ++j) {
                D2 e[4], r2[4], d[3];
                UKFB_UNROLL
                for (int i = 0; i < 4; ++i) {
                    const double x = UKFB_PS(PF_E + 4 * j + i);
                    e[i] = D2(x, i < 3 ? -x : x);
                }
                quat_mul(e, c, r2);
                pf_log(r2, d, slow);
                UKFB_UNROLL
                for (int r = 0; r < 3; ++r) {
                    UKFB_UNROLL
                    for (int cc = 0; cc < 3; ++cc) S[r * 3 + cc] = fma(d[r].a, d[cc].a, fma(d[r].b, d[cc].b, S[r * 3 + cc]));
                    UKFB_PS(PF_E + 4 * j + r) = d[r].a - d[r].b;
                }
            }
            double r4[4];
            quat_mul_conj(zin, zref, r4);
            pf_log(r4, innov, slow);
        }
        if (slow) return false;
        UKFB_UNROLL
        for (int r = 0; r < 3; ++r) {
            UKFB_UNROLL
            for (int cc = 0; cc < 3; ++cc) S[r * 3 + cc] = fma(0.5, S[r * 3 + cc], Rmeas[r * r_ld + cc]);
        }
        UKFB_UNROLL
        for (int i = 0; i < 36; ++i) Sxz[i] = 0.0;
        UKFB_UNROLL
        for (int j = 0; j < 6; ++j) {
            UKFB_UNROLL
            for (int cc = 0; cc < 3; ++cc) {
                const double ddz = UKFB_PS(PF_E + 4 * j + cc);
                UKFB_UNROLL
                for (int i = j; i < 12; ++i) Sxz[i * 3 + cc] = fma(a[tri(i, j)], ddz, Sxz[i * 3 + cc]);
            }
        }
        UKFB_UNROLL
        for (int i = 0; i < 36; ++i) Sxz[i] *= 0.5;
    } else {
    UKFB_UNROLL
    for (int c = 0; c < 3; ++c) {
        const int s = sel[c] < 0 ? 0 : sel[c];
        const bool used = c < m_dim;
        UKFB_UNROLL
        for (int i = 0; i < 12; ++i) {
            const int e = i >= s ? tri(i, 0) + s : tri(s, 0) + i;
            const double x = UKFB_PS(e);
            Sxz[i * 3 + c] = used ? x : 0.0;
        }
        innov[c] = used ? zm[c] - pf_mu_tangent(m, s) : 0.0;
    }
    UKFB_UNROLL
    for (int a = 0; a < 3; ++a) {
        UKFB_UNROLL
        for (int c = 0; c < 3; ++c) {
            const int sa = sel[a] < 0 ? 0 : sel[a], sc = sel[c] < 0 ? 0 : sel[c];
            const int e = sa >= sc ? tri(sa, 0) + sc : tri(sc, 0) + sa;
            const bool used = a < m_dim && c < m_dim;
            const double x = UKFB_PS(e);
            S[a * 3 + c] = used ? x + Rmeas[a * r_ld + c] : (a == c ? 1.0 : 0.0);
        }
    }
    }
    double Si[9];
    {
        const double c00 = S[4] * S[8] - S[5] * S[7];
        const double c10 = S[7] * S[2] - S[8] * S[1];
        const double c20 = S[1] * S[5] - S[2] * S[4];
        const double det = c00 * S[0] + c10 * S[3] + c20 * S[6];
        const double invdet = 1.0 / det;
        Si[0] = c00 * invdet;
        Si[1] = c10 * invdet;
        Si[2] = c20 * invdet;
        Si[3] = (S[5] * S[6] - S[3] * S[8]) * invdet;
        Si[4] = (S[8] * S[0] - S[6] * S[2]) * invdet;
        Si[5] = (S[2] * S[3] - S[0] * S[5]) * invdet;
        Si[6] = (S[3] * S[7] - S[4] * S[6]) * invdet;
        Si[7] = (S[6] * S[1] - S[7] * S[0]) * invdet;
        Si[8] = (S[0] * S[4] - S[1] * S[3]) * invdet;
    }
    {
        double d2 = 0.0;
        UKFB_UNROLL
        for (int a = 0; a < 3; ++a) d2 += innov[a] * (Si[a * 3] * innov[0] + Si[a * 3 + 1] * innov[1] + Si[a * 3 + 2] * innov[2]);
        if (d2 > gate_d2) {
            status |= UKFB_STATUS_MEAS_REJECTED;
            return true;
        }
    }
    double a[PoseF::LP];
    UKFB_UNROLL
    for (int i = 0; i < 12; ++i) {
        double k3[3], ks3[3];
        UKFB_UNROLL
        for (int cc = 0; cc < 3; ++cc) {
            double s = 0.0;
            UKFB_UNROLL
            for (int k = 0; k < 3; ++k) s += Sxz[i * 3 + k] * Si[k * 3 + cc];
            k3[cc] = s;
        }
        double dl = 0.0;
        UKFB_UNROLL
        for (int c = 0; c < 3; ++c) {
            ks3[c] = Sxz[i * 3 + c];
            Sxz[i * 3 + c] = k3[c];
            dl += k3[c] * innov[c];
        }
        delta[i] = dl;
        UKFB_UNROLL
        for (int j = 0; j <= i; ++j) {
            double s = 0.0;
            UKFB_UNROLL
            for (int k = 0; k < 3; ++k) s += ks3[k] * Sxz[j * 3 + k];
            const double x = UKFB_PS(tri(i, j)) - s;
            a[tri(i, j)] = x;
            sig[tri(i, j) * TILE] = x;
        }
    }
    stage = 1;
    const bool wide_trace = a[tri(3, 3)] + a[tri(4, 4)] + a[tri(5, 5)] > PF_WIDE_TRACE;
    spd = pf_cholesky<6>(a);
    if (!spd) return true;
    UKFB_UNROLL
    for (int j = 0; j < 6; ++j) {
        UKFB_UNROLL
        for (int i = 0; i < 12; ++i) UKFB_PS(PF_LA + j * 12 + i) = i >= j ? a[tri(i, j)] : 0.0;
    }

    if (wide_trace) {
        stage = 2;
        return false;
    }
    return pf_apply_delta<false>(sm, lane, sig, m, delta, status, passes_out, stage);
}

template <bool WITH_ORI>
UKFB_DNI PfLit pf_update_slow(double* sm, int lane, double* sig, int kind, const double* zm, const double* Rm, int r_ld, ModelArgs ma,
                              PoseMu m, PfDelta delta, int stage, double gate_d2)
{
    if (WITH_ORI && stage == 0 && kind == UKFB_MEAS_POSE_ORIENTATION) {
        UKFB_UNROLL
        for (int e = 0; e < PoseF::LP; ++e) UKFB_PS(e) = sig[e * TILE];
        const double tr = UKFB_PS(tri(3, 3)) + UKFB_PS(tri(4, 4)) + UKFB_PS(tri(5, 5));
        if (tr < PF_PI2_GUARD) {
            PfLit r;
            r.m = m, r.status = 0, r.passes = 0;
            bool spd = true;
            const bool done = pf_update<true>(sm, lane, sig, kind, zm, Rm, r_ld, r.m, delta.d, r.status, r.passes, spd, gate_d2, stage);
            if (done) {
                if (!spd) r.status |= UKFB_STATUS_NOT_SPD;
                return r;
            }
        }
    }
    if (stage == 0 && kind != UKFB_MEAS_POSE_ORIENTATION) {
        double a[PoseF::LP];
        UKFB_UNROLL
        for (int e = 0; e < PoseF::LP; ++e) a[e] = UKFB_PS(e);
        bool ok = pf_cholesky<6>(a);
        UKFB_UNROLL
        for (int j = 0; j < 6; ++j) {
            double n2 = a[tri(5, j)] * a[tri(5, j)];
            if (j <= 4) n2 += a[tri(4, j)] * a[tri(4, j)];
            if (j <= 3) n2 += a[tri(3, j)] * a[tri(3, j)];
            ok = ok && n2 < PF_PI2_COLUMN;
        }
        if (ok) {
            PfLit r;
            r.m = m, r.status = 0, r.passes = 0;
            bool spd = true;
            if (pf_update<false>(sm, lane, sig, kind, zm, Rm, r_ld, r.m, delta.d, r.status, r.passes, spd, gate_d2, stage)) {
                if (!spd) r.status |= UKFB_STATUS_NOT_SPD;
                return r;
            }
        }
    }
    if (stage == 2) {
        PfLit r;
        r.m = m, r.status = 0, r.passes = 0;
        if (pf_apply_delta<true>(sm, lane, sig, r.m, delta.d, r.status, r.passes, stage)) {
            UKFB_PF_COUNT(4);
            return r;
        }
        stage = 1;
    }
    return pf_literal_update(sig, kind, zm, Rm, r_ld, ma, m, delta, stage == 0, gate_d2);
}

template <bool WITH_ORI, bool OVERLAP = false>
UKFB_GLOBAL void UKFB_LAUNCH_BOUNDS(UKFB_PF_MAX_THREADS, UKFB_PF_MIN_BLOCKS) ukf_pose_fast_kernel(const UKFB_GRID_CONSTANT StepParams p)
{
    typedef PoseF F;
    UKFB_SMEM_DECL
    const int lane = threadIdx.x & 31, wib = threadIdx.x >> 5;
    const long long tile = (long long)blockIdx.x * (blockDim.x >> 5) + wib;
    double* sm = ukfb_smem + wib * (PF_PER_LANE * TILE);
    if (OVERLAP) pdl_launch_dependents();
    if (tile * TILE >= p.B) return;
    if (OVERLAP) tile_done_wait(p.tile_done + tile, 32ull * (p.launch_seq - 1));
    const long long b = tile * TILE + lane;
    const bool valid = b < p.B;
    const long long bb = valid ? b : p.B - 1;
    double* rec = p.state + tile * (TILE * F::REC) + lane;
    double* sig = rec + F::MU * TILE;

    PoseMu m;
    UKFB_UNROLL
    for (int i = 0; i < 3; ++i) m.p[i] = rec[i * TILE], m.v[i] = rec[(7 + i) * TILE], m.w[i] = rec[(10 + i) * TILE];
    UKFB_UNROLL
    for (int i = 0; i < 4; ++i) m.q[i] = rec[(3 + i) * TILE];
    prefetch_next_wave<F>(p, tile, lane);

    ModelArgs ma;
    ma.dt = 0.0;
    ma.has_acc = false;
    ma.neg_inv_tau_g = 0.0;
    ma.neg_inv_tau_a = 0.0;
    UKFB_UNROLL
    for (int i = 0; i < 3; ++i) {
        ma.earth[i] = 0.0;
        ma.acc[i] = p.acc_mu[bb * 3 + i];
        ma.omega[i] = 0.0;
    }
    const double big = 1.79769313486231570e308;
    uint32_t status = 0;
    bool dirty_mu = false;
    int hist[8] = {0, 0, 0, 0, 0, 0, 0, 0};

    UKFB_NOUNROLL
    for (int tick = 0; tick < p.K; ++tick) {
        double a[F::LP];
        UKFB_UNROLL
        for (int e = 0; e < F::LP; ++e) a[e] = sig[e * TILE];

        bool do_pred = false, do_upd = false;
        int kind = -1, store = -1;
        const double* Rmeas = p.R + tick * p.r_kstride + b * p.r_stride;
        if (valid) {
            bool idle = false;
            if (p.events) {
                kind = int(p.kinds[tick * p.kinds_kstride + b]);
                idle = kind == UKFB_EVENT_IDLE;
                if (kind < UKFB_EVENT_IDLE || kind == UKFB_MEAS_ORI_VELOCITY || kind > UKFB_EVENT_POSE_ACCELERATION) {
                    status |= UKFB_STATUS_BAD_EVENT;
                    idle = true;
                }
                if (idle) kind = -1;
                if (kind >= 0) Rmeas += kind * p.r_kind_stride;
                if (kind == UKFB_EVENT_POSE_ACCELERATION) store = kind, kind = -1;
            }
            if (p.do_predict && !idle) {
                double dt;
                bool have_dt = true;
                if (p.time_mode) {
                    const long long ts = p.ts[tick * p.ts_kstride + b * p.ts_stride];
                    const long long tl = p.t_last[b];
                    if (tl == 0) {
                        p.t_last[b] = ts;
                        have_dt = false;
                        dt = 0.0;
                    } else {
                        dt = double(ts - tl) / UKFB_US_PER_S;
                        if (dt > p.min_dt) p.t_last[b] = ts;
                    }
                } else {
                    dt = p.dt[tick * p.dt_kstride + b * p.dt_stride];
                }
                if (have_dt) {
                    if (dt < 0.0) {
                        status |= UKFB_STATUS_NEG_DT;
                        if (p.events) kind = -1, store = -1;
                    } else if (dt <= p.min_dt) {
                    } else if (dt > p.max_dt) {
                        status |= UKFB_STATUS_DT_TOO_LARGE;
                        if (p.events) kind = -1, store = -1;
                    }
                    else {
                        do_pred = true;
                        ma.dt = dt;
                    }
                }
            }
            if (p.do_update && !idle) {
                if (!p.events) {
                    kind = p.tick_kinds ? int(p.tick_kinds[tick]) : (p.kind == -2 ? int(p.kinds[tick * p.kinds_kstride + b]) : p.kind);
                    if (p.kind == -2 && !p.tick_kinds && kind != UKFB_MEAS_NONE && !meas_kind_of_class<F>(kind)) {
                        status |= UKFB_STATUS_BAD_EVENT;
                        kind = -1;
                    }
                    if (p.mask && !p.mask[tick * p.mask_kstride + b]) kind = -1;
                }
                do_upd = kind >= 0;
            }
        }

        int passes_a = 0, passes_b = 0;
        bool sigma_in_smem = false;
        const double* Qp = p.Q + b * p.q_stride;
        const double* acov = p.acc_cov ? p.acc_cov + b * 9 : nullptr;

        if (do_pred) {
            ma.has_acc = (fabs(ma.acc[0]) <= big) && (fabs(ma.acc[1]) <= big) && (fabs(ma.acc[2]) <= big);
            bool spd = true;
            const bool want_smem = do_upd && kind != UKFB_MEAS_POSE_ORIENTATION;
            if (pf_predict<false>(p.q_diagonal, sm, lane, sig, a, Qp, acov, ma, m, want_smem, status, passes_a, spd)) {
                if (!spd) {
                    status |= UKFB_STATUS_NOT_SPD;
                    do_upd = false;
                } else {
                    sigma_in_smem = want_smem;
                    dirty_mu = true;
                }
            } else {
                int in_smem = 0;
                const PfLit r = pf_predict_slow(sm, lane, sig, Qp, acov, ma, m, want_smem ? 1 : 0, p.q_diagonal, &in_smem);
                status |= r.status;
                passes_a = r.passes;
                if (r.status & UKFB_STATUS_NOT_SPD)
                    do_upd = false;
                else {
                    m = r.m;
                    sigma_in_smem = in_smem != 0;
                    dirty_mu = true;
                }
            }
        }

        if (store >= 0) {
            const double* zm = p.z + tick * p.z_kstride + b * p.z_stride;
            UKFB_UNROLL
            for (int r = 0; r < 3; ++r) {
                ma.acc[r] = zm[r];
                UKFB_UNROLL
                for (int cc = 0; cc < 3; ++cc) p.acc_cov[b * 9 + r * 3 + cc] = Rmeas[r * p.r_ld + cc];
            }
        }

        if (do_upd) {
            const double* zm = p.z + tick * p.z_kstride + b * p.z_stride;
            bool literal = kind == UKFB_MEAS_POSE_ORIENTATION;
            if (!literal) {
                if (!sigma_in_smem) {
                    double a2[F::LP];
                    UKFB_UNROLL
                    for (int e = 0; e < F::LP; ++e) a2[e] = sig[e * TILE];
                    UKFB_UNROLL
                    for (int e = 0; e < F::LP; ++e) UKFB_PS(e) = a2[e];
                    if (!pf_cholesky<12>(a2)) {
                        status |= UKFB_STATUS_NOT_SPD;
                        do_upd = false;
                    }
                }
                const double tr = UKFB_PS(tri(3, 3)) + UKFB_PS(tri(4, 4)) + UKFB_PS(tri(5, 5));
                literal = !(tr < PF_PI2_GUARD);
            }
            if (do_upd) {
                bool spd = true, fast_done = false;
                int stage = 0;
                double delta[12];
                UKFB_UNROLL
                for (int i = 0; i < 12; ++i) delta[i] = 0.0;
                if (!literal) {
                    fast_done = pf_update<false>(sm, lane, sig, kind, zm, Rmeas, p.r_ld, m, delta, status, passes_b, spd, p.gate_d2, stage);
                    if (fast_done) {
                        if (!spd)
                            status |= UKFB_STATUS_NOT_SPD;
                        else
                            dirty_mu = true;
                    }
                }
                if (!fast_done) {
                    PfDelta dl;
                    UKFB_UNROLL
                    for (int i = 0; i < 12; ++i) dl.d[i] = delta[i];
                    const PfLit r = pf_update_slow<WITH_ORI>(sm, lane, sig, kind, zm, Rmeas, p.r_ld, ma, m, dl, literal ? 0 : stage, p.gate_d2);
                    status |= r.status;
                    passes_b = r.passes;
                    if (!(r.status & UKFB_STATUS_NOT_SPD)) {
                        m = r.m;
                        dirty_mu = true;
                    }
                }
            }
        }
        {
            const int pa = passes_a < 7 ? passes_a : 7, pb = passes_b < 7 ? passes_b : 7;
            UKFB_UNROLL
            for (int k = 1; k < 8; ++k) hist[k] += (pa == k) + (pb == k);
        }
    }

    if (valid && dirty_mu) {
        UKFB_UNROLL
        for (int i = 0; i < 3; ++i) rec[i * TILE] = m.p[i], rec[(7 + i) * TILE] = m.v[i], rec[(10 + i) * TILE] = m.w[i];
        UKFB_UNROLL
        for (int i = 0; i < 4; ++i) rec[(3 + i) * TILE] = m.q[i];
    }
    if (valid && p.events) {
        UKFB_UNROLL
        for (int i = 0; i < 3; ++i) p.acc_mu[b * 3 + i] = ma.acc[i];
    }
    if (valid && status) p.status[b] |= status;
    if (p.hist && valid) {
        unsigned long long* hs = p.hist + (tile % HIST_SLOTS) * 8;
        UKFB_UNROLL
        for (int k = 1; k < 8; ++k)
            if (hist[k]) atomicAdd(hs + k, (unsigned long long)hist[k]);
    }
    if (OVERLAP) tile_done_add(p.tile_done + tile);
}

#undef UKFB_PS

}

#endif
```

Before: 1.197 billion.

## Cache sigma-point propagation results in tensor memory across mean iterations

Splits sigma-point propagation from the reference-difference step. On the first mean-iteration pass, the propagated quaternions and exponentials are stored in Blackwell tensor memory (tcgen05), and positions go to shared memory. Later passes reload them instead of recomputing the exp and quaternion products. To make the whole warp take the cached path together, it adds warp votes and moves the loop exit into a warp-uniform form. It also fixes the pose kernel at 4 warps per block, with TMEM allocation, fences and block barriers. The cost is extra synchronisation and TMEM allocation per block, and lanes that have already converged may keep running iterations.

```diff
diff --git a/slam_pose_estimation_b200/csrc/simt.cuh b/slam_pose_estimation_b200/csrc/simt.cuh
--- a/slam_pose_estimation_b200/csrc/simt.cuh
+++ b/slam_pose_estimation_b200/csrc/simt.cuh
@@ -28,6 +28,49 @@
 
 UKFB_D double warp_shfl(double v, int src) { return __shfl_sync(0xffffffffu, v, src); }
 
+UKFB_D bool warp_all(bool p) { return __all_sync(0xffffffffu, p); }
+UKFB_D bool warp_any(bool p) { return __any_sync(0xffffffffu, p); }
+UKFB_D void block_sync() { __syncthreads(); }
+
+constexpr int TMEM_COLS = 256;
+__shared__ uint32_t ukfb_tmem_slot;
+UKFB_D void tmem_alloc()
+{
+    asm volatile("tcgen05.alloc.cta_group::1.sync.aligned.shared::cta.b32 [%0], %1;" ::"r"(uint32_t(__cvta_generic_to_shared(&ukfb_tmem_slot))),
+                 "r"(uint32_t(TMEM_COLS))
+                 : "memory");
+    asm volatile("tcgen05.relinquish_alloc_permit.cta_group::1.sync.aligned;" ::: "memory");
+}
+UKFB_D void tmem_dealloc()
+{
+    asm volatile("tcgen05.dealloc.cta_group::1.sync.aligned.b32 %0, %1;" ::"r"(ukfb_tmem_slot), "r"(uint32_t(TMEM_COLS)) : "memory");
+}
+UKFB_D uint32_t tmem_warp_base() { return ukfb_tmem_slot + ((threadIdx.x & 0x60u) << 16); }
+UKFB_D void tmem_fence_before() { asm volatile("tcgen05.fence::before_thread_sync;" ::: "memory"); }
+UKFB_D void tmem_fence_after() { asm volatile("tcgen05.fence::after_thread_sync;" ::: "memory"); }
+UKFB_D void tmem_store8(uint32_t taddr, const double* v)
+{
+    asm volatile("tcgen05.st.sync.aligned.32x32b.x16.b32 [%0], {%1,%2,%3,%4,%5,%6,%7,%8,%9,%10,%11,%12,%13,%14,%15,%16};" ::"r"(taddr),
+                 "r"(__double2loint(v[0])), "r"(__double2hiint(v[0])), "r"(__double2loint(v[1])), "r"(__double2hiint(v[1])),
+                 "r"(__double2loint(v[2])), "r"(__double2hiint(v[2])), "r"(__double2loint(v[3])), "r"(__double2hiint(v[3])),
+                 "r"(__double2loint(v[4])), "r"(__double2hiint(v[4])), "r"(__double2loint(v[5])), "r"(__double2hiint(v[5])),
+                 "r"(__double2loint(v[6])), "r"(__double2hiint(v[6])), "r"(__double2loint(v[7])), "r"(__double2hiint(v[7]))
+                 : "memory");
+}
+UKFB_D void tmem_wait_st() { asm volatile("tcgen05.wait::st.sync.aligned;" ::: "memory"); }
+UKFB_D void tmem_load8(uint32_t taddr, double* v)
+{
+    int w[16];
+    asm volatile("tcgen05.ld.sync.aligned.32x32b.x16.b32 {%0,%1,%2,%3,%4,%5,%6,%7,%8,%9,%10,%11,%12,%13,%14,%15}, [%16];\n\t"
+                 "tcgen05.wait::ld.sync.aligned;"
+                 : "=r"(w[0]), "=r"(w[1]), "=r"(w[2]), "=r"(w[3]), "=r"(w[4]), "=r"(w[5]), "=r"(w[6]), "=r"(w[7]), "=r"(w[8]),
+                   "=r"(w[9]), "=r"(w[10]), "=r"(w[11]), "=r"(w[12]), "=r"(w[13]), "=r"(w[14]), "=r"(w[15])
+                 : "r"(taddr)
+                 : "memory");
+    UKFB_UNROLL
+    for (int i = 0; i < 8; ++i) v[i] = __hiloint2double(w[2 * i + 1], w[2 * i]);
+}
+
 UKFB_D int hi_word(double x) { return __double2hiint(x); }
 
 UKFB_D void pdl_launch_dependents() { asm volatile("griddepcontrol.launch_dependents;" ::: "memory"); }
@@ -92,8 +135,12 @@
 
 #else
 
+#include <atomic>
 #include <cmath>
 #include <cstdint>
+#include <cstdio>
+#include <cstdlib>
+#include <cstring>
 
 #include "simt_emu_rt.hpp"
 
@@ -145,6 +192,56 @@
     __syncwarp();
     return r;
 }
+inline bool warp_vote(bool p, bool all)
+{
+    double* x = ::simt_emu::warp_xchg();
+    x[threadIdx.x & 31] = p ? 1.0 : 0.0;
+    __syncwarp();
+    bool r = all;
+    for (int l = 0; l < 32; ++l) r = all ? (r && x[l] != 0.0) : (r || x[l] != 0.0);
+    __syncwarp();
+    return r;
+}
+inline bool warp_all(bool p) { return warp_vote(p, true); }
+inline bool warp_any(bool p) { return warp_vote(p, false); }
+inline void block_sync()
+{
+    if (blockDim.x > 32) {
+        std::fprintf(stderr, "simt emulation: block barrier in a block of more than one warp\n");
+        std::abort();
+    }
+    __syncwarp();
+}
+constexpr int TMEM_COLS = 256;
+inline thread_local uint32_t tmem_lane[TMEM_COLS];
+inline std::atomic<unsigned long long> tmem_accesses{0};
+inline void tmem_alloc() { __syncwarp(); }
+inline void tmem_dealloc() { __syncwarp(); }
+inline uint32_t tmem_warp_base() { return (threadIdx.x & 0x60u) << 16; }
+inline void tmem_fence_before() {}
+inline void tmem_fence_after() {}
+inline void tmem_wait_st() {}
+inline uint32_t* tmem_cells(uint32_t taddr, int ncols)
+{
+    const unsigned col = taddr & 0xffffu;
+    if ((taddr >> 16) != (threadIdx.x & 0x60u) || int(col) + ncols > TMEM_COLS) {
+        std::fprintf(stderr, "simt emulation: tensor-memory address 0x%08x outside the warp's lanes or columns\n", taddr);
+        std::abort();
+    }
+    double* x = ::simt_emu::warp_xchg();
+    x[threadIdx.x & 31] = double(taddr);
+    __syncwarp();
+    for (int l = 0; l < 32; ++l)
+        if (x[l] != double(taddr)) {
+            std::fprintf(stderr, "simt emulation: tensor-memory access 0x%08x not issued by the whole warp together\n", taddr);
+            std::abort();
+        }
+    __syncwarp();
+    tmem_accesses.fetch_add(1, std::memory_order_relaxed);
+    return tmem_lane + col;
+}
+inline void tmem_store8(uint32_t taddr, const double* v) { std::memcpy(tmem_cells(taddr, 16), v, 8 * sizeof(double)); }
+inline void tmem_load8(uint32_t taddr, double* v) { std::memcpy(v, tmem_cells(taddr, 16), 8 * sizeof(double)); }
 inline void warp_dmma(double& c0, double& c1, double a, double b)
 {
     double* x = ::simt_emu::warp_xchg();
@@ -167,6 +264,11 @@
 }
 }
 
-#endif
-
-#endif
+extern "C" __attribute__((used, visibility("default"))) inline unsigned long long ukfb_emu_tmem_accesses(void)
+{
+    return ukfb::tmem_accesses.load();
+}
+
+#endif
+
+#endif
diff --git a/slam_pose_estimation_b200/csrc/ukf_batch.cu b/slam_pose_estimation_b200/csrc/ukf_batch.cu
--- a/slam_pose_estimation_b200/csrc/ukf_batch.cu
+++ b/slam_pose_estimation_b200/csrc/ukf_batch.cu
@@ -658,10 +658,9 @@
 }
 
 template <class K>
-static cudaError_t launch_fast(K kernel, K kernel_overlap, int per_lane, ukfb_handle* h, const StepParams& p, ukfb_handle::FastCfg& cfg)
+static cudaError_t launch_fast(K kernel, K kernel_overlap, int per_lane, int wpb, ukfb_handle* h, const StepParams& p, ukfb_handle::FastCfg& cfg)
 {
     const EnvKnobs& kn = knobs();
-    const int wpb = kn.fast_wpb;
     const size_t smem = sizeof(double) * per_lane * TILE * wpb + size_t(kn.smem_pad_kb) * 1024;
     if (!cfg.attr_set) {
         cudaError_t e = ensure_smem_attr(kernel, h->device, smem);
@@ -709,14 +708,16 @@
 
 static cudaError_t launch_pose_fast(ukfb_handle* h, const StepParams& p, bool may_have_orientation_meas)
 {
-    if (may_have_orientation_meas) return launch_fast(ukf_pose_fast_kernel<true, false>, ukf_pose_fast_kernel<true, true>, PF_PER_LANE, h, p, h->fast_cfg[1]);
-    return launch_fast(ukf_pose_fast_kernel<false, false>, ukf_pose_fast_kernel<false, true>, PF_PER_LANE, h, p, h->fast_cfg[0]);
+    if (may_have_orientation_meas)
+        return launch_fast(ukf_pose_fast_kernel<true, false>, ukf_pose_fast_kernel<true, true>, PF_PER_LANE, PF_WPB, h, p, h->fast_cfg[1]);
+    return launch_fast(ukf_pose_fast_kernel<false, false>, ukf_pose_fast_kernel<false, true>, PF_PER_LANE, PF_WPB, h, p, h->fast_cfg[0]);
 }
 
 static cudaError_t launch_ori_fast(ukfb_handle* h, const StepParams& p)
 {
-    if (p.ori_params) return launch_fast(ukf_ori_fast_kernel<true, false>, ukf_ori_fast_kernel<true, true>, OF_PER_LANE, h, p, h->fast_cfg[1]);
-    return launch_fast(ukf_ori_fast_kernel<false, false>, ukf_ori_fast_kernel<false, true>, OF_PER_LANE, h, p, h->fast_cfg[0]);
+    const int wpb = knobs().fast_wpb;
+    if (p.ori_params) return launch_fast(ukf_ori_fast_kernel<true, false>, ukf_ori_fast_kernel<true, true>, OF_PER_LANE, wpb, h, p, h->fast_cfg[1]);
+    return launch_fast(ukf_ori_fast_kernel<false, false>, ukf_ori_fast_kernel<false, true>, OF_PER_LANE, wpb, h, p, h->fast_cfg[0]);
 }
 
 static int launch_step(ukfb_handle* h, const StepParams& p)
diff --git a/slam_pose_estimation_b200/csrc/ukf_pose_fast.cuh b/slam_pose_estimation_b200/csrc/ukf_pose_fast.cuh
--- a/slam_pose_estimation_b200/csrc/ukf_pose_fast.cuh
+++ b/slam_pose_estimation_b200/csrc/ukf_pose_fast.cuh
@@ -376,25 +376,59 @@
 }
 
 
+enum PfCache { PF_EVAL = 0, PF_STORE = 1, PF_LOAD = 2 };
+constexpr uint32_t PF_TM_A = 0, PF_TM_B = 96;
+static_assert(PF_TM_B + 6 * 16 <= TMEM_COLS, "tensor-memory columns of the pose kernel");
+UKFB_D void pf_tm_store(uint32_t col, const D2* q)
+{
+    const double v[8] = {q[0].a, q[0].b, q[1].a, q[1].b, q[2].a, q[2].b, q[3].a, q[3].b};
+    tmem_store8(tmem_warp_base() + col, v);
+}
+UKFB_D void pf_tm_load(uint32_t col, D2* q)
+{
+    double v[8];
+    tmem_load8(tmem_warp_base() + col, v);
+    UKFB_UNROLL
+    for (int i = 0; i < 4; ++i) q[i] = D2(v[2 * i], v[2 * i + 1]);
+}
+
 template <bool WIDE>
-UKFB_D void pf_point2(const D2* qs, const D2* ps, const D2* vs, const D2* ws, double dt, const double* ref_p, const double* ref_q,
-                      D2* d, bool& slow)
-{
-    D2 rv[3], e[4], qn[4], r[4];
+UKFB_D void pf_propagate2(const D2* qs, const D2* ps, const D2* vs, const D2* ws, double dt, D2* pn, D2* qn, bool& slow)
+{
+    D2 rv[3], e[4];
     pf_rotate(qs, vs, rv);
     pf_exp_t<WIDE>(ws, dt, e, slow);
     quat_mul(qs, e, qn);
-    d[0] = tfma(dt, rv[0], ps[0]) - ref_p[0];
-    d[1] = tfma(dt, rv[1], ps[1]) - ref_p[1];
-    d[2] = tfma(dt, rv[2], ps[2]) - ref_p[2];
+    pn[0] = tfma(dt, rv[0], ps[0]);
+    pn[1] = tfma(dt, rv[1], ps[1]);
+    pn[2] = tfma(dt, rv[2], ps[2]);
+}
+
+template <bool WIDE>
+UKFB_D void pf_minus_ref2(const D2* pn, const D2* qn, const double* ref_p, const double* ref_q, D2* d, bool& slow)
+{
+    D2 r[4];
+    d[0] = pn[0] - ref_p[0];
+    d[1] = pn[1] - ref_p[1];
+    d[2] = pn[2] - ref_p[2];
     quat_mul_conj(qn, ref_q, r);
     pf_log_t<WIDE>(r, d + 3, slow);
 }
 
 template <bool WIDE>
-UKFB_D void pf_pair_a(const double* sm, int lane, int j, const PoseMu& m, const double* vm, double dt, const double* ref_p,
-                      const double* ref_q, double* L, double* dpl, double* dmi, bool& slow)
-{
+UKFB_D void pf_pair_a(double* sm, int lane, int j, const PoseMu& m, const double* vm, double dt, const double* ref_p,
+                      const double* ref_q, double* L, double* dpl, double* dmi, bool& slow, int cache = PF_EVAL)
+{
+    D2 pn[3], qn[4], d[6];
+    if (cache == PF_LOAD) {
+        pf_tm_load(PF_TM_A + 16 * j, qn);
+        UKFB_UNROLL
+        for (int i = 0; i < 3; ++i) pn[i] = D2(UKFB_PS(PF_LA + j * 12 + i), UKFB_PS(PF_LA + j * 12 + 3 + i));
+        pf_minus_ref2<WIDE>(pn, qn, ref_p, ref_q, d, slow);
+        UKFB_UNROLL
+        for (int i = 0; i < 6; ++i) dpl[i] = d[i].a, dmi[i] = d[i].b;
+        return;
+    }
     UKFB_UNROLL
     for (int i = 0; i < 12; ++i) L[i] = UKFB_PS(PF_LA + j * 12 + i);
     double e[4];
@@ -409,25 +443,36 @@
     const D2 ps[3] = {D2(m.p[0] + L[0], m.p[0] - L[0]), D2(m.p[1] + L[1], m.p[1] - L[1]), D2(m.p[2] + L[2], m.p[2] - L[2])};
     const D2 vs[3] = {D2(vm[0] + L[6], vm[0] - L[6]), D2(vm[1] + L[7], vm[1] - L[7]), D2(vm[2] + L[8], vm[2] - L[8])};
     const D2 ws[3] = {D2(m.w[0] + L[9], m.w[0] - L[9]), D2(m.w[1] + L[10], m.w[1] - L[10]), D2(m.w[2] + L[11], m.w[2] - L[11])};
-    D2 d[6];
-    pf_point2<WIDE>(qs, ps, vs, ws, dt, ref_p, ref_q, d, slow);
+    pf_propagate2<WIDE>(qs, ps, vs, ws, dt, pn, qn, slow);
+    if (cache == PF_STORE) {
+        pf_tm_store(PF_TM_A + 16 * j, qn);
+        UKFB_UNROLL
+        for (int i = 0; i < 3; ++i) UKFB_PS(PF_LA + j * 12 + i) = pn[i].a, UKFB_PS(PF_LA + j * 12 + 3 + i) = pn[i].b;
+    }
+    pf_minus_ref2<WIDE>(pn, qn, ref_p, ref_q, d, slow);
     UKFB_UNROLL
     for (int i = 0; i < 6; ++i) dpl[i] = d[i].a, dmi[i] = d[i].b;
 }
 
 template <bool WIDE>
 UKFB_D void pf_pair_b(const double* sm, int lane, int j, const double* Rm, const double* rw0, const double* c, double dt,
-                      double* L, double* dopl, double* domi, double* wv, bool& slow)
+                      double* L, double* dopl, double* domi, double* wv, bool& slow, int cache = PF_EVAL)
 {
     UKFB_UNROLL
     for (int i = 0; i < 6; ++i) L[i] = UKFB_PS(PF_LB + (j - 6) * 6 + i);
-    double u[3], rv[3];
-    pf_matvec(Rm, L + 3, u);
+    double rv[3];
     pf_matvec(Rm, L, rv);
     wv[0] = dt * rv[0], wv[1] = dt * rv[1], wv[2] = dt * rv[2];
-    const D2 rw[3] = {D2(rw0[0] + u[0], rw0[0] - u[0]), D2(rw0[1] + u[1], rw0[1] - u[1]), D2(rw0[2] + u[2], rw0[2] - u[2])};
     D2 e[4], r[4], d[3];
-    pf_exp_t<WIDE>(rw, dt, e, slow);
+    if (cache == PF_LOAD) {
+        pf_tm_load(PF_TM_B + 16 * (j - 6), e);
+    } else {
+        double u[3];
+        pf_matvec(Rm, L + 3, u);
+        const D2 rw[3] = {D2(rw0[0] + u[0], rw0[0] - u[0]), D2(rw0[1] + u[1], rw0[1] - u[1]), D2(rw0[2] + u[2], rw0[2] - u[2])};
+        pf_exp_t<WIDE>(rw, dt, e, slow);
+        if (cache == PF_STORE) pf_tm_store(PF_TM_B + 16 * (j - 6), e);
+    }
     quat_mul(e, c, r);
     pf_log_t<WIDE>(r, d, slow);
     UKFB_UNROLL
@@ -435,15 +480,21 @@
 }
 
 template <bool WIDE>
-UKFB_D void pf_pair_d(const double* sm, int lane, int j, const double* delta, const double* c, double* dp, double* dn, bool& slow)
+UKFB_D void pf_pair_d(const double* sm, int lane, int j, const double* delta, const double* c, double* dp, double* dn, bool& slow,
+                      int cache = PF_EVAL)
 {
     D2 v[3], e[4], r2[4], d[3];
-    UKFB_UNROLL
-    for (int i = 0; i < 3; ++i) {
-        const double l = UKFB_PS(PF_LA + j * 12 + 3 + i);
-        v[i] = D2(delta[3 + i] + l, delta[3 + i] - l);
-    }
-    pf_exp_t<WIDE>(v, 1.0, e, slow);
+    if (cache == PF_LOAD) {
+        pf_tm_load(PF_TM_A + 16 * j, e);
+    } else {
+        UKFB_UNROLL
+        for (int i = 0; i < 3; ++i) {
+            const double l = UKFB_PS(PF_LA + j * 12 + 3 + i);
+            v[i] = D2(delta[3 + i] + l, delta[3 + i] - l);
+        }
+        pf_exp_t<WIDE>(v, 1.0, e, slow);
+        if (cache == PF_STORE) pf_tm_store(PF_TM_A + 16 * j, e);
+    }
     quat_mul(e, c, r2);
     pf_log_t<WIDE>(r2, d, slow);
     UKFB_UNROLL
@@ -455,11 +506,11 @@
 #endif
 constexpr double PF_WIDE_COLUMN_N2 = UKFB_PF_WIDE_COLUMN_N2;
 template <bool WIDE>
-UKFB_D void pf_pair_a_sel(const double* sm, int lane, int j, const PoseMu& m, const double* vm, double dt, const double* ref_p,
-                          const double* ref_q, double* L, double* dpl, double* dmi, bool& slow)
+UKFB_D void pf_pair_a_sel(double* sm, int lane, int j, const PoseMu& m, const double* vm, double dt, const double* ref_p,
+                          const double* ref_q, double* L, double* dpl, double* dmi, bool& slow, int cache)
 {
     if (!WIDE) {
-        pf_pair_a<false>(sm, lane, j, m, vm, dt, ref_p, ref_q, L, dpl, dmi, slow);
+        pf_pair_a<false>(sm, lane, j, m, vm, dt, ref_p, ref_q, L, dpl, dmi, slow, cache);
         return;
     }
     const double l3 = UKFB_PS(PF_LA + j * 12 + 3), l4 = UKFB_PS(PF_LA + j * 12 + 4), l5 = UKFB_PS(PF_LA + j * 12 + 5);
@@ -469,10 +520,10 @@
 }
 template <bool WIDE>
 UKFB_D void pf_pair_b_sel(const double* sm, int lane, int j, const double* Rm, const double* rw0, const double* c, double dt,
-                          double* L, double* dopl, double* domi, double* wv, bool& slow)
+                          double* L, double* dopl, double* domi, double* wv, bool& slow, int cache)
 {
     if (!WIDE) {
-        pf_pair_b<false>(sm, lane, j, Rm, rw0, c, dt, L, dopl, domi, wv, slow);
+        pf_pair_b<false>(sm, lane, j, Rm, rw0, c, dt, L, dopl, domi, wv, slow, cache);
         return;
     }
     bool redo = false;
@@ -480,10 +531,11 @@
     if (redo) pf_pair_b<true>(sm, lane, j, Rm, rw0, c, dt, L, dopl, domi, wv, slow);
 }
 template <bool WIDE>
-UKFB_D void pf_pair_d_sel(const double* sm, int lane, int j, const double* delta, const double* c, double* dp, double* dn, bool& slow)
+UKFB_D void pf_pair_d_sel(const double* sm, int lane, int j, const double* delta, const double* c, double* dp, double* dn, bool& slow,
+                          int cache)
 {
     if (!WIDE) {
-        pf_pair_d<false>(sm, lane, j, delta, c, dp, dn, slow);
+        pf_pair_d<false>(sm, lane, j, delta, c, dp, dn, slow, cache);
         return;
     }
     const double l3 = UKFB_PS(PF_LA + j * 12 + 3), l4 = UKFB_PS(PF_LA + j * 12 + 4), l5 = UKFB_PS(PF_LA + j * 12 + 5);
@@ -587,12 +639,15 @@
 
 template <bool WIDE>
 UKFB_D bool pf_predict(int q_diagonal, double* sm, int lane, double* sig, double* a, const double* Qp, const double* acov,
-                       const ModelArgs& ma, PoseMu& m, bool to_smem, uint32_t& status, int& passes_out, bool& spd)
+                       const ModelArgs& ma, PoseMu& m, bool to_smem, uint32_t& status, int& passes_out, bool& spd, bool tm = false)
 {
     const double dt = ma.dt;
-    if (!WIDE && a[tri(3, 3)] + a[tri(4, 4)] + a[tri(5, 5)] > PF_WIDE_TRACE) return false;
+    const bool wide = !WIDE && a[tri(3, 3)] + a[tri(4, 4)] + a[tri(5, 5)] > PF_WIDE_TRACE;
+    tm = !WIDE && tm && warp_all(!wide);
+    if (wide) return false;
     {
         spd = pf_cholesky<12>(a);
+        tm = tm && warp_all(spd);
         if (!spd) return true;
         UKFB_UNROLL
         for (int j = 0; j < 6; ++j) {
@@ -629,21 +684,24 @@
     double ref_q[4] = {q0n[0], q0n[1], q0n[2], q0n[3]};
 
     int it = 0, passes = 0;
+    bool active = true;
+    int cache = tm ? PF_STORE : PF_EVAL;
     while (true) {
+        bool ps = slow;
         double md[6];
         double d0[6];
         {
             double r[4];
             d0[0] = p0n[0] - ref_p[0], d0[1] = p0n[1] - ref_p[1], d0[2] = p0n[2] - ref_p[2];
             quat_mul_conj(q0n, ref_q, r);
-            pf_log1<WIDE>(r, d0 + 3, slow);
+            pf_log1<WIDE>(r, d0 + 3, ps);
         }
         md[0] = 13.0 * d0[0], md[1] = 13.0 * d0[1], md[2] = 13.0 * d0[2];
         md[3] = d0[3], md[4] = d0[4], md[5] = d0[5];
         UKFB_LOOP_UNROLL(UKFB_PF_MEAN_UNROLL)
         for (int j = 0; j < 6; ++j) {
             double L[12], dpl[6], dmi[6];
-            pf_pair_a_sel<WIDE>(sm, lane, j, m, vm, dt, ref_p, ref_q, L, dpl, dmi, slow);
+            pf_pair_a_sel<WIDE>(sm, lane, j, m, vm, dt, ref_p, ref_q, L, dpl, dmi, ps, cache);
             UKFB_UNROLL
             for (int i = 0; i < 6; ++i) md[i] += dpl[i] + dmi[i];
         }
@@ -652,31 +710,40 @@
         UKFB_LOOP_UNROLL(UKFB_PF_MEAN_UNROLL)
         for (int j = 6; j < 12; ++j) {
             double L[6], dopl[3], domi[3], wv[3];
-            pf_pair_b_sel<WIDE>(sm, lane, j, Rm, rw0, c, dt, L, dopl, domi, wv, slow);
+            pf_pair_b_sel<WIDE>(sm, lane, j, Rm, rw0, c, dt, L, dopl, domi, wv, ps, cache);
             UKFB_UNROLL
             for (int i = 0; i < 3; ++i) md[3 + i] += dopl[i] + domi[i];
         }
-        double n2 = 0.0;
-        UKFB_UNROLL
-        for (int i = 0; i < 6; ++i) {
-            md[i] = div_ns<PoseF::NS>(md[i]);
-            n2 += md[i] * md[i];
-        }
-        ref_p[0] += md[0], ref_p[1] += md[1], ref_p[2] += md[2];
-        {
-            double e[4], r[4];
-            pf_exp1<WIDE>(md + 3, 1.0, e, slow);
-            quat_mul(e, ref_q, r);
-            ref_q[0] = r[0], ref_q[1] = r[1], ref_q[2] = r[2], ref_q[3] = r[3];
-        }
-        ++passes;
-        if (slow || !(n2 > UKFB_MEAN_TOL * UKFB_MEAN_TOL)) break;
-        if (++it >= UKFB_MEAN_MAX_IT) {
-            status |= UKFB_STATUS_MEAN_NO_CONVERGE;
-            break;
-        }
-    }
-    if (slow) return false;
+        if (cache == PF_STORE) {
+            tmem_wait_st();
+            cache = PF_LOAD;
+        }
+        if (active) {
+            slow = ps;
+            double n2 = 0.0;
+            UKFB_UNROLL
+            for (int i = 0; i < 6; ++i) {
+                md[i] = div_ns<PoseF::NS>(md[i]);
+                n2 += md[i] * md[i];
+            }
+            ref_p[0] += md[0], ref_p[1] += md[1], ref_p[2] += md[2];
+            {
+                double e[4], r[4];
+                pf_exp1<WIDE>(md + 3, 1.0, e, slow);
+                quat_mul(e, ref_q, r);
+                ref_q[0] = r[0], ref_q[1] = r[1], ref_q[2] = r[2], ref_q[3] = r[3];
+            }
+            ++passes;
+            if (slow || !(n2 > UKFB_MEAN_TOL * UKFB_MEAN_TOL))
+                active = false;
+            else if (++it >= UKFB_MEAN_MAX_IT) {
+                status |= UKFB_STATUS_MEAN_NO_CONVERGE;
+                active = false;
+            }
+        }
+        if (!(tm ? warp_any(active) : active)) break;
+    }
+    if (slow && !tm) return false;
 
     double C[21], X[36];
     {
@@ -692,7 +759,7 @@
         UKFB_LOOP_UNROLL(UKFB_PF_COV_UNROLL)
         for (int j = 0; j < 6; ++j) {
             double L[12], dpl[6], dmi[6];
-            pf_pair_a_sel<WIDE>(sm, lane, j, m, vm, dt, ref_p, ref_q, L, dpl, dmi, slow);
+            pf_pair_a_sel<WIDE>(sm, lane, j, m, vm, dt, ref_p, ref_q, L, dpl, dmi, slow, cache);
             UKFB_UNROLL
             for (int i = 0; i < 6; ++i) {
                 UKFB_UNROLL
@@ -709,7 +776,7 @@
         UKFB_LOOP_UNROLL(UKFB_PF_COV_UNROLL)
         for (int j = 6; j < 12; ++j) {
             double L[6], dpl[6], dmi[6], wv[3];
-            pf_pair_b_sel<WIDE>(sm, lane, j, Rm, rw0, c, dt, L, dpl + 3, dmi + 3, wv, slow);
+            pf_pair_b_sel<WIDE>(sm, lane, j, Rm, rw0, c, dt, L, dpl + 3, dmi + 3, wv, slow, cache);
             UKFB_UNROLL
             for (int i = 0; i < 3; ++i) dpl[i] = d0[i] + wv[i], dmi[i] = d0[i] - wv[i];
             UKFB_UNROLL
@@ -883,7 +950,8 @@
 }
 
 template <bool WIDE>
-UKFB_D bool pf_apply_delta(double* sm, int lane, double* sig, PoseMu& m, const double* delta, uint32_t& status, int& passes_out, int& stage)
+UKFB_D bool pf_apply_delta(double* sm, int lane, double* sig, PoseMu& m, const double* delta, uint32_t& status, int& passes_out, int& stage,
+                           bool tm = false)
 {
     bool slow = !pf_unit(m.q);
     const bool off_sphere = slow;
@@ -893,39 +961,52 @@
     quat_mul(e0, m.q, q0n);
     double ref_q[4] = {q0n[0], q0n[1], q0n[2], q0n[3]};
     int it = 0, passes = 0;
+    bool active = true;
+    int cache = tm ? PF_STORE : PF_EVAL;
     while (true) {
+        bool ps = slow;
         double c[4], r[4], d0[3], md[3];
         quat_mul_conj(m.q, ref_q, c);
         quat_mul(e0, c, r);
-        pf_log1<WIDE>(r, d0, slow);
+        pf_log1<WIDE>(r, d0, ps);
         md[0] = 13.0 * d0[0], md[1] = 13.0 * d0[1], md[2] = 13.0 * d0[2];
         UKFB_NOUNROLL
         for (int j = 0; j < 6; ++j) {
             double dp[3], dn[3];
-            pf_pair_d_sel<WIDE>(sm, lane, j, delta, c, dp, dn, slow);
+            pf_pair_d_sel<WIDE>(sm, lane, j, delta, c, dp, dn, ps, cache);
             md[0] += dp[0] + dn[0], md[1] += dp[1] + dn[1], md[2] += dp[2] + dn[2];
         }
-        double n2 = 0.0;
-        UKFB_UNROLL
-        for (int i = 0; i < 3; ++i) {
-            md[i] = div_ns<PoseF::NS>(md[i]);
-            n2 += md[i] * md[i];
-        }
-        {
-            double e[4], rr[4];
-            pf_exp1<WIDE>(md, 1.0, e, slow);
-            quat_mul(e, ref_q, rr);
-            ref_q[0] = rr[0], ref_q[1] = rr[1], ref_q[2] = rr[2], ref_q[3] = rr[3];
-        }
-        ++passes;
-        if (slow || !(n2 > UKFB_MEAN_TOL * UKFB_MEAN_TOL)) break;
-        if (++it >= UKFB_MEAN_MAX_IT) {
-            status |= UKFB_STATUS_MEAN_NO_CONVERGE;
-            break;
-        }
+        if (cache == PF_STORE) {
+            tmem_wait_st();
+            cache = PF_LOAD;
+        }
+        if (active) {
+            slow = ps;
+            double n2 = 0.0;
+            UKFB_UNROLL
+            for (int i = 0; i < 3; ++i) {
+                md[i] = div_ns<PoseF::NS>(md[i]);
+                n2 += md[i] * md[i];
+            }
+            {
+                double e[4], rr[4];
+                pf_exp1<WIDE>(md, 1.0, e, slow);
+                quat_mul(e, ref_q, rr);
+                ref_q[0] = rr[0], ref_q[1] = rr[1], ref_q[2] = rr[2], ref_q[3] = rr[3];
+            }
+            ++passes;
+            if (slow || !(n2 > UKFB_MEAN_TOL * UKFB_MEAN_TOL))
+                active = false;
+            else if (++it >= UKFB_MEAN_MAX_IT) {
+                status |= UKFB_STATUS_MEAN_NO_CONVERGE;
+                active = false;
+            }
+        }
+        if (!(tm ? warp_any(active) : active)) break;
     }
     double Coo[6], Xc[27];
-    if (!slow) {
+    const bool slow_mean = slow;
+    if (tm || !slow) {
         double c[4], r[4], d0[3];
         quat_mul_conj(m.q, ref_q, c);
         quat_mul(e0, c, r);
@@ -939,17 +1020,19 @@
         UKFB_NOUNROLL
         for (int j = 0; j < 6; ++j) {
             double dp[3], dn[3];
-            pf_pair_d_sel<WIDE>(sm, lane, j, delta, c, dp, dn, late);
+            pf_pair_d_sel<WIDE>(sm, lane, j, delta, c, dp, dn, late, cache);
             UKFB_UNROLL
             for (int i = 0; i < 3; ++i) {
                 UKFB_UNROLL
                 for (int k = 0; k <= i; ++k) Coo[tri(i, k)] = fma(dp[i], dp[k], fma(dn[i], dn[k], Coo[tri(i, k)]));
             }
-            UKFB_UNROLL
-            for (int k = 0; k < 3; ++k) UKFB_PS(PF_LA + j * 12 + 3 + k) = dp[k] - dn[k];
+            if (!slow_mean) {
+                UKFB_UNROLL
+                for (int k = 0; k < 3; ++k) UKFB_PS(PF_LA + j * 12 + 3 + k) = dp[k] - dn[k];
+            }
         }
         slow = slow || late;
-        lost_factor = late;
+        lost_factor = late && !slow_mean;
         UKFB_UNROLL
         for (int i = 0; i < 27; ++i) Xc[i] = 0.0;
         UKFB_UNROLL
@@ -993,7 +1076,7 @@
 
 template <bool ORI_MEAS>
 UKFB_D bool pf_update(double* sm, int lane, double* sig, int kind, const double* zm, const double* Rmeas, int r_ld, PoseMu& m,
-                      double* delta, uint32_t& status, int& passes_out, bool& spd, double gate_d2, int& stage)
+                      double* delta, uint32_t& status, int& passes_out, bool& spd, double gate_d2, int& stage, bool tm = false)
 {
     stage = 0;
     const int m_dim = meas_dim(kind);
@@ -1152,6 +1235,7 @@
         double d2 = 0.0;
         UKFB_UNROLL
         for (int a = 0; a < 3; ++a) d2 += innov[a] * (Si[a * 3] * innov[0] + Si[a * 3 + 1] * innov[1] + Si[a * 3 + 2] * innov[2]);
+        tm = tm && warp_all(!(d2 > gate_d2));
         if (d2 > gate_d2) {
             status |= UKFB_STATUS_MEAS_REJECTED;
             return true;
@@ -1189,6 +1273,7 @@
     stage = 1;
     const bool wide_trace = a[tri(3, 3)] + a[tri(4, 4)] + a[tri(5, 5)] > PF_WIDE_TRACE;
     spd = pf_cholesky<6>(a);
+    tm = tm && warp_all(spd && !wide_trace);
     if (!spd) return true;
     UKFB_UNROLL
     for (int j = 0; j < 6; ++j) {
@@ -1200,7 +1285,7 @@
         stage = 2;
         return false;
     }
-    return pf_apply_delta<false>(sm, lane, sig, m, delta, status, passes_out, stage);
+    return pf_apply_delta<false>(sm, lane, sig, m, delta, status, passes_out, stage, tm);
 }
 
 template <bool WITH_ORI>
@@ -1256,17 +1341,10 @@
     return pf_literal_update(sig, kind, zm, Rm, r_ld, ma, m, delta, stage == 0, gate_d2);
 }
 
-template <bool WITH_ORI, bool OVERLAP = false>
-UKFB_GLOBAL void UKFB_LAUNCH_BOUNDS(UKFB_PF_MAX_THREADS, UKFB_PF_MIN_BLOCKS) ukf_pose_fast_kernel(const UKFB_GRID_CONSTANT StepParams p)
+template <bool WITH_ORI, bool OVERLAP>
+UKFB_D void pf_tile(const StepParams& p, long long tile, int lane, double* sm)
 {
     typedef PoseF F;
-    UKFB_SMEM_DECL
-    const int lane = threadIdx.x & 31, wib = threadIdx.x >> 5;
-    const long long tile = (long long)blockIdx.x * (blockDim.x >> 5) + wib;
-    double* sm = ukfb_smem + wib * (PF_PER_LANE * TILE);
-    if (OVERLAP) pdl_launch_dependents();
-    if (tile * TILE >= p.B) return;
-    if (OVERLAP) tile_done_wait(p.tile_done + tile, 32ull * (p.launch_seq - 1));
     const long long b = tile * TILE + lane;
     const bool valid = b < p.B;
     const long long bb = valid ? b : p.B - 1;
@@ -1368,11 +1446,12 @@
         const double* Qp = p.Q + b * p.q_stride;
         const double* acov = p.acc_cov ? p.acc_cov + b * 9 : nullptr;
 
+        const bool tm_pred = warp_all(do_pred);
         if (do_pred) {
             ma.has_acc = (fabs(ma.acc[0]) <= big) && (fabs(ma.acc[1]) <= big) && (fabs(ma.acc[2]) <= big);
             bool spd = true;
             const bool want_smem = do_upd && kind != UKFB_MEAS_POSE_ORIENTATION;
-            if (pf_predict<false>(p.q_diagonal, sm, lane, sig, a, Qp, acov, ma, m, want_smem, status, passes_a, spd)) {
+            if (pf_predict<false>(p.q_diagonal, sm, lane, sig, a, Qp, acov, ma, m, want_smem, status, passes_a, spd, tm_pred)) {
                 if (!spd) {
                     status |= UKFB_STATUS_NOT_SPD;
                     do_upd = false;
@@ -1405,9 +1484,8 @@
             }
         }
 
+        bool literal = kind == UKFB_MEAS_POSE_ORIENTATION;
         if (do_upd) {
-            const double* zm = p.z + tick * p.z_kstride + b * p.z_stride;
-            bool literal = kind == UKFB_MEAS_POSE_ORIENTATION;
             if (!literal) {
                 if (!sigma_in_smem) {
                     double a2[F::LP];
@@ -1423,14 +1501,19 @@
                 const double tr = UKFB_PS(tri(3, 3)) + UKFB_PS(tri(4, 4)) + UKFB_PS(tri(5, 5));
                 literal = !(tr < PF_PI2_GUARD);
             }
-            if (do_upd) {
+        }
+        const bool tm_upd = warp_all(do_upd && !literal);
+        if (do_upd) {
+            const double* zm = p.z + tick * p.z_kstride + b * p.z_stride;
+            {
                 bool spd = true, fast_done = false;
                 int stage = 0;
                 double delta[12];
                 UKFB_UNROLL
                 for (int i = 0; i < 12; ++i) delta[i] = 0.0;
                 if (!literal) {
-                    fast_done = pf_update<false>(sm, lane, sig, kind, zm, Rmeas, p.r_ld, m, delta, status, passes_b, spd, p.gate_d2, stage);
+                    fast_done = pf_update<false>(sm, lane, sig, kind, zm, Rmeas, p.r_ld, m, delta, status, passes_b, spd, p.gate_d2, stage,
+                                                 tm_upd);
                     if (fast_done) {
                         if (!spd)
                             status |= UKFB_STATUS_NOT_SPD;
@@ -1479,6 +1562,32 @@
     if (OVERLAP) tile_done_add(p.tile_done + tile);
 }
 
+constexpr int PF_WPB = 4;
+template <bool WITH_ORI, bool OVERLAP = false>
+UKFB_GLOBAL void UKFB_LAUNCH_BOUNDS(UKFB_PF_MAX_THREADS, UKFB_PF_MIN_BLOCKS) ukf_pose_fast_kernel(const UKFB_GRID_CONSTANT StepParams p)
+{
+    UKFB_SMEM_DECL
+    const int lane = threadIdx.x & 31, wib = threadIdx.x >> 5;
+    const long long tile = (long long)blockIdx.x * (blockDim.x >> 5) + wib;
+    const bool live = tile * TILE < p.B;
+    if (OVERLAP) {
+        pdl_launch_dependents();
+        if (live) tile_done_wait(p.tile_done + tile, 32ull * (p.launch_seq - 1));
+        block_sync();
+    }
+    if (wib == 0) tmem_alloc();
+    tmem_fence_before();
+    block_sync();
+    tmem_fence_after();
+    if (live) pf_tile<WITH_ORI, OVERLAP>(p, tile, lane, ukfb_smem + wib * (PF_PER_LANE * TILE));
+    tmem_fence_before();
+    block_sync();
+    if (wib == 0) {
+        tmem_fence_after();
+        tmem_dealloc();
+    }
+}
+
 #undef UKFB_PS
 
 }
```

Result: slower. 1.142 billion, median of 6 (-4.5%).
